# kyleliang919/distributed-lion-pytorch

Measured on AMD Instinct MI355X. Metric: tokens/sec + all-reduce bytes/step, GPT-2 CLM at 1/2/4/8 MI355X, higher is better.
Workload: dtype bf16; 1 GPU; model=gpt2 (124.4M params), trainable_params=124439808, base_weights=bf16, global_batch=160, task=clm, gradient_checkpointing=False, micro_batch=20, grad_accum=8, seq_len=1024, parallelism=dp1, optimizer=distributed Lion (majority vote), lr 0.0001, wd 0.1, exchange=a2a, impl=native

## Files before the change

### distributed_lion_pytorch_amd/csrc/bindings.cpp

```cpp
#include <ATen/ATen.h>
#include <c10/core/DeviceGuard.h>
#include <c10/hip/HIPStream.h>
#include <torch/library.h>

#include <hip/hip_runtime.h>

#include <cstdlib>
#include <string>
#include <tuple>
#include <vector>

#include "kernels.h"

namespace dlion {
enum class Layout : int { NT = 0, NN = 1, TN = 2, TT = 3 };
bool lt_gemm(const void* a, int64_t lda, const void* b, int64_t ldb, void* c, int64_t ldc, const void* bias,
             int64_t M, int64_t N, int64_t K, int epi, int device, hipStream_t s, Layout lay, bool accumulate);
}

namespace {

using at::Tensor;

void check_dev(const Tensor& t, const char* name) {
  TORCH_CHECK(t.is_cuda(), "dlion: ", name, " must be a GPU (HIP) tensor");
  TORCH_CHECK(t.is_contiguous(), "dlion: ", name, " must be contiguous");
}

void check_hip(hipError_t e, const char* what) {
  TORCH_CHECK(e == hipSuccess, "dlion: ", what, " failed: ", hipGetErrorString(e));
}

hipStream_t cur_stream() { return c10::hip::getCurrentHIPStream().stream(); }

const float* gscale_ptr(const std::optional<Tensor>& gscale) {
  if (!gscale.has_value()) return nullptr;
  check_dev(*gscale, "gscale");
  TORCH_CHECK(gscale->scalar_type() == at::kFloat && gscale->numel() >= 2, "dlion: gscale must be float32[2]");
  return gscale->data_ptr<float>();
}

void check_rounding(int64_t rounding, int64_t dtype, int64_t coord_base) {
  TORCH_CHECK(rounding == 0 || rounding == 1, "dlion: bad parameter rounding mode ", rounding);
  TORCH_CHECK(rounding == 0 || dtype != 2, "dlion: stochastic parameter rounding does not support fp16");
  TORCH_CHECK(coord_base >= 0 && coord_base % 8 == 0, "dlion: the coordinate base must be a multiple of 8");
}

void lion_local(const Tensor& meta, int64_t seg_off, int64_t chunk_off, int64_t n_chunks, int64_t dtype,
                double decay, double neg_lr, double b1, double omb1, double b2, double omb2,
                const std::optional<Tensor>& gscale, int64_t rounding, int64_t rkey, int64_t coord_base) {
  check_dev(meta, "meta");
  TORCH_CHECK(meta.scalar_type() == at::kLong, "dlion: meta must be int64");
  check_rounding(rounding, dtype, coord_base);
  const c10::DeviceGuard g(meta.device());
  const int64_t* base = meta.data_ptr<int64_t>();
  check_hip(dlion::launch_lion_local(static_cast<int>(dtype), base + seg_off, base + chunk_off, n_chunks,
                                     static_cast<float>(decay), static_cast<float>(neg_lr), static_cast<float>(b1),
                                     static_cast<float>(omb1), static_cast<float>(b2), static_cast<float>(omb2),
                                     gscale_ptr(gscale), cur_stream(), static_cast<int>(rounding),
                                     static_cast<uint32_t>(rkey), coord_base),
            "lion_local");
}

void lion_encode(const Tensor& meta, int64_t seg_off, int64_t chunk_off, int64_t n_chunks, int64_t dtype,
                 const Tensor& bits, double b1, double omb1, double b2, double omb2, bool update_m,
                 bool stochastic, double rr, int64_t seed, int64_t step, const std::optional<Tensor>& gscale,
                 int64_t cbase) {
  check_dev(meta, "meta");
  check_dev(bits, "bits");
  TORCH_CHECK(bits.scalar_type() == at::kByte, "dlion: bits must be uint8");
  TORCH_CHECK(cbase >= 0 && cbase % 8 == 0, "dlion: the coordinate base must be a multiple of 8");
  const c10::DeviceGuard g(meta.device());
  const int64_t* base = meta.data_ptr<int64_t>();
  check_hip(dlion::launch_lion_encode(static_cast<int>(dtype), base + seg_off, base + chunk_off, n_chunks,
                                      bits.data_ptr<uint8_t>(), static_cast<float>(b1), static_cast<float>(omb1),
                                      static_cast<float>(b2), static_cast<float>(omb2), update_m ? 1 : 0,
                                      stochastic ? 1 : 0, static_cast<float>(rr), static_cast<uint64_t>(seed),
                                      static_cast<uint32_t>(step), gscale_ptr(gscale), cur_stream(), cbase),
            "lion_encode");
}

void grad_sumsq(const Tensor& meta, int64_t seg_off, int64_t chunk_off, int64_t n_chunks, int64_t dtype,
                const Tensor& partial, int64_t part_off) {
  check_dev(meta, "meta");
  check_dev(partial, "partial");
  TORCH_CHECK(partial.scalar_type() == at::kFloat && part_off + n_chunks <= partial.numel(),
              "dlion: grad_sumsq partial buffer too small");
  const c10::DeviceGuard g(meta.device());
  const int64_t* base = meta.data_ptr<int64_t>();
  check_hip(dlion::launch_grad_sumsq(static_cast<int>(dtype), base + seg_off, base + chunk_off, n_chunks,
                                     partial.data_ptr<float>() + part_off, cur_stream()),
            "grad_sumsq");
}

void clip_coef(const Tensor& partial, int64_t n, double max_norm, const Tensor& out) {
  check_dev(partial, "partial");
  check_dev(out, "out");
  TORCH_CHECK(partial.scalar_type() == at::kFloat && out.scalar_type() == at::kFloat && out.numel() >= 2 &&
                  n <= partial.numel(),
              "dlion: clip_coef needs float32 partials and a float32[2] output");
  const c10::DeviceGuard g(partial.device());
  check_hip(dlion::launch_clip_coef(partial.data_ptr<float>(), n, static_cast<float>(max_norm), out.data_ptr<float>(),
                                    cur_stream()),
            "clip_coef");
}

void lion_vote_apply(const Tensor& meta, int64_t seg_off, int64_t chunk_off, int64_t n_chunks, int64_t dtype,
                     const Tensor& planes, int64_t plane_stride, const Tensor& alive, int64_t mode, int64_t tie,
                     const std::optional<Tensor>& neg, double decay, double neg_lr,
                     const std::optional<Tensor>& own, const std::optional<Tensor>& agree, int64_t rounding,
                     int64_t rkey, int64_t coord_base) {
  check_dev(meta, "meta");
  check_rounding(rounding, dtype, coord_base);
  check_dev(planes, "planes");
  check_dev(alive, "alive");
  TORCH_CHECK(planes.scalar_type() == at::kByte, "dlion: planes must be uint8");
  TORCH_CHECK(alive.scalar_type() == at::kByte, "dlion: alive must be uint8");
  TORCH_CHECK(mode >= 0 && mode <= 3, "dlion: bad vote mode ", mode);
  if (mode == 3) {
    const int64_t w = alive.numel();
    TORCH_CHECK(w >= 1 && w <= 15, "dlion: counted apply needs 1 <= W <= 15, got ", w);
    int64_t p = 0;
    while (w >> p) ++p;
    TORCH_CHECK(plane_stride > 0 && plane_stride % 256 == 0, "dlion: counted apply shard bytes must be a multiple of 256");
    TORCH_CHECK(planes.numel() >= w * p * plane_stride, "dlion: counted apply count planes too small");
  }
  const uint8_t* negp = nullptr;
  if (neg.has_value()) {
    check_dev(*neg, "neg");
    negp = neg->data_ptr<uint8_t>();
  }
  unsigned long long* agp = nullptr;
  const uint8_t* ownp = nullptr;
  if (agree.has_value()) {
    TORCH_CHECK(own.has_value(), "dlion: vote agreement needs this rank's own bits");
    check_dev(*own, "own");
    ownp = own->data_ptr<uint8_t>();
    check_dev(*agree, "agree");
    TORCH_CHECK(agree->scalar_type() == at::kLong && agree->numel() >= 2,
                "dlion: agree must be int64 [agreements, ties]");
    agp = reinterpret_cast<unsigned long long*>(agree->data_ptr<int64_t>());
  }
  const c10::DeviceGuard g(meta.device());
  const int64_t* base = meta.data_ptr<int64_t>();
  check_hip(dlion::launch_lion_vote_apply(static_cast<int>(dtype), base + seg_off, base + chunk_off, n_chunks,
                                          planes.data_ptr<uint8_t>(), plane_stride, alive.data_ptr<uint8_t>(),
                                          static_cast<int>(alive.numel()), static_cast<int>(mode),
                                          static_cast<int>(tie), negp, static_cast<float>(decay),
                                          static_cast<float>(neg_lr), ownp, agp, cur_stream(),
                                          static_cast<int>(rounding), static_cast<uint32_t>(rkey), coord_base),
            "lion_vote_apply");
}

void vote_reduce(const Tensor& recv, int64_t nbytes, const Tensor& alive, int64_t tie, const Tensor& out,
                 const std::optional<Tensor>& neg_out, const std::optional<Tensor>& ties) {
  check_dev(recv, "recv");
  check_dev(alive, "alive");
  check_dev(out, "out");
  TORCH_CHECK(nbytes % 4 == 0, "dlion: vote_reduce shard bytes must be a multiple of 4");
  TORCH_CHECK(out.numel() >= nbytes, "dlion: vote_reduce out too small");
  TORCH_CHECK(recv.numel() >= nbytes * alive.numel(), "dlion: vote_reduce recv too small");
  uint8_t* negp = nullptr;
  if (neg_out.has_value()) {
    check_dev(*neg_out, "neg_out");
    negp = neg_out->data_ptr<uint8_t>();
  }
  unsigned long long* tp = nullptr;
  if (ties.has_value()) {
    check_dev(*ties, "ties");
    TORCH_CHECK(ties->scalar_type() == at::kLong && ties->numel() >= 1, "dlion: ties must be int64");
    tp = reinterpret_cast<unsigned long long*>(ties->data_ptr<int64_t>());
  }
  const c10::DeviceGuard g(recv.device());
  check_hip(dlion::launch_vote_reduce(recv.data_ptr<uint8_t>(), nbytes, alive.data_ptr<uint8_t>(),
                                      static_cast<int>(alive.numel()), static_cast<int>(tie),
                                      out.data_ptr<uint8_t>(), negp, tp, cur_stream()),
            "vote_reduce");
}

void vote_count(const Tensor& recv, int64_t nbytes, const Tensor& alive, const Tensor& out,
                const std::optional<Tensor>& ties) {
  check_dev(recv, "recv");
  check_dev(alive, "alive");
  check_dev(out, "out");
  TORCH_CHECK(recv.scalar_type() == at::kByte && out.scalar_type() == at::kByte && alive.scalar_type() == at::kByte,
              "dlion: vote_count buffers must be uint8");
  const int64_t w = alive.numel();
  TORCH_CHECK(w >= 1 && w <= 15, "dlion: vote_count needs 1 <= W <= 15, got ", w);
  int64_t p = 0;
  while (w >> p) ++p;
  TORCH_CHECK(nbytes >= 0 && nbytes % 4 == 0, "dlion: vote_count shard bytes must be a multiple of 4");
  TORCH_CHECK(out.numel() >= p * nbytes, "dlion: vote_count out too small");
  TORCH_CHECK(recv.numel() >= nbytes * w, "dlion: vote_count recv too small");
  unsigned long long* tp = nullptr;
  if (ties.has_value()) {
    check_dev(*ties, "ties");
    TORCH_CHECK(ties->scalar_type() == at::kLong && ties->numel() >= 1, "dlion: ties must be int64");
    tp = reinterpret_cast<unsigned long long*>(ties->data_ptr<int64_t>());
  }
  const c10::DeviceGuard g(recv.device());
  check_hip(dlion::launch_vote_count(recv.data_ptr<uint8_t>(), nbytes, alive.data_ptr<uint8_t>(),
                                     static_cast<int>(w), out.data_ptr<uint8_t>(), tp, cur_stream()),
            "vote_count");
}

int dtype_code(at::ScalarType t) {
  switch (t) {
    case at::kFloat: return 0;
    case at::kBFloat16: return 1;
    case at::kHalf: return 2;
    default: TORCH_CHECK(false, "dlion: unsupported dtype ", t);
  }
  return -1;
}

Tensor softmax_xent_(const Tensor& logits, const Tensor& labels, int64_t v, int64_t variant) {
  check_dev(logits, "logits");
  check_dev(labels, "labels");
  TORCH_CHECK(logits.dim() == 2, "dlion: logits must be [N, Vpad]");
  TORCH_CHECK(labels.scalar_type() == at::kLong && labels.numel() == logits.size(0), "dlion: labels must be int64[N]");
  TORCH_CHECK(logits.size(1) % 8 == 0 && v <= logits.size(1), "dlion: padded vocab must be a multiple of 8");
  const c10::DeviceGuard g(logits.device());
  auto loss = at::empty({logits.size(0)}, logits.options().dtype(at::kFloat));
  check_hip(dlion::launch_softmax_xent(dtype_code(logits.scalar_type()), logits.data_ptr(), labels.data_ptr<int64_t>(),
                                       logits.size(0), logits.size(1), static_cast<int>(v), loss.data_ptr<float>(),
                                       static_cast<int>(variant), cur_stream()),
            "softmax_xent");
  return loss;
}

Tensor softmax_xent_opts_(const Tensor& logits, const Tensor& labels, int64_t v, double smoothing, double z_loss,
                          int64_t variant) {
  check_dev(logits, "logits");
  check_dev(labels, "labels");
  TORCH_CHECK(logits.dim() == 2 && logits.is_contiguous(), "dlion: logits must be a contiguous [N, Vpad]");
  TORCH_CHECK(labels.scalar_type() == at::kLong && labels.numel() == logits.size(0) && labels.is_contiguous(),
              "dlion: labels must be int64[N]");
  TORCH_CHECK(logits.size(1) % 8 == 0 && v > 0 && v <= logits.size(1), "dlion: padded vocab must be a multiple of 8");
  TORCH_CHECK(smoothing >= 0.0 && smoothing < 1.0 && z_loss >= 0.0, "dlion: need 0 <= smoothing < 1 and z_loss >= 0");
  const c10::DeviceGuard g(logits.device());
  auto loss = at::empty({logits.size(0)}, logits.options().dtype(at::kFloat));
  check_hip(dlion::launch_softmax_xent_opts(dtype_code(logits.scalar_type()), logits.data_ptr(),
                                            labels.data_ptr<int64_t>(), logits.size(0), logits.size(1),
                                            static_cast<int>(v), loss.data_ptr<float>(), static_cast<float>(smoothing),
                                            static_cast<float>(z_loss), static_cast<int>(variant), cur_stream()),
            "softmax_xent_opts");
  return loss;
}

std::tuple<Tensor, Tensor, Tensor, Tensor> lm_score(const Tensor& logits, const Tensor& labels, int64_t v,
                                                    double smoothing, double z_loss) {
  check_dev(logits, "logits");
  check_dev(labels, "labels");
  TORCH_CHECK(logits.dim() == 2 && logits.is_contiguous(), "dlion: logits must be a contiguous [N, Vpad]");
  TORCH_CHECK(labels.scalar_type() == at::kLong && labels.numel() == logits.size(0) && labels.is_contiguous(),
              "dlion: labels must be int64[N]");
  TORCH_CHECK(logits.size(1) % 8 == 0 && v > 0 && v <= logits.size(1), "dlion: padded vocab must be a multiple of 8");
  TORCH_CHECK(logits.size(1) <= (int64_t{1} << 30), "dlion: lm_score vocabulary too wide");
  TORCH_CHECK(smoothing >= 0.0 && smoothing < 1.0 && z_loss >= 0.0, "dlion: need 0 <= smoothing < 1 and z_loss >= 0");
  const c10::DeviceGuard g(logits.device());
  const int64_t n = logits.size(0);
  auto loss = at::empty({n}, logits.options().dtype(at::kFloat));
  auto lse = at::empty({n}, logits.options().dtype(at::kFloat));
  auto pred = at::empty({n}, logits.options().dtype(at::kInt));
  auto rank = at::empty({n}, logits.options().dtype(at::kInt));
  check_hip(dlion::launch_lm_score(dtype_code(logits.scalar_type()), logits.data_ptr(), labels.data_ptr<int64_t>(), n,
                                   logits.size(1), static_cast<int>(v), static_cast<float>(smoothing),
                                   static_cast<float>(z_loss), loss.data_ptr<float>(), lse.data_ptr<float>(),
                                   pred.data_ptr<int>(), rank.data_ptr<int>(), cur_stream()),
            "lm_score");
  return {loss, lse, pred, rank};
}

void check_bthd(const Tensor& t, const char* name) {
  TORCH_CHECK(t.is_cuda() && t.scalar_type() == at::kBFloat16, "dlion attn: ", name, " must be a bf16 GPU tensor");
  TORCH_CHECK(t.dim() == 4 && t.stride(3) == 1, "dlion attn: ", name, " must be [B,T,H,D] with contiguous D");
  TORCH_CHECK(reinterpret_cast<uintptr_t>(t.data_ptr()) % 16 == 0 && t.stride(1) % 8 == 0 && t.stride(2) % 8 == 0 &&
                  t.stride(0) % 8 == 0,
              "dlion attn: ", name, " must be 16-byte aligned");
}

dlion::AttnArgs attn_args(const Tensor& q, const Tensor& k, const Tensor& v, double p, int64_t seed) {
  check_bthd(q, "q");
  check_bthd(k, "k");
  check_bthd(v, "v");
  const int64_t B = q.size(0), T = q.size(1), H = q.size(2), D = q.size(3), Hkv = k.size(2);
  TORCH_CHECK(k.size(0) == B && k.size(1) == T && k.size(3) == D && v.sizes() == k.sizes(), "dlion attn: shape mismatch");
  TORCH_CHECK(H % Hkv == 0, "dlion attn: H must be a multiple of Hkv");
  TORCH_CHECK(T >= 1 && (D == 64 || D == 128), "dlion attn: need T >= 1 and D in {64, 128}");
  TORCH_CHECK(p >= 0.0 && p < 1.0, "dlion attn: dropout must be in [0, 1)");
  dlion::AttnArgs a{};
  a.q = static_cast<const __bf16*>(q.data_ptr());
  a.k = static_cast<const __bf16*>(k.data_ptr());
  a.v = static_cast<const __bf16*>(v.data_ptr());
  a.q_sb = q.stride(0); a.q_st = q.stride(1); a.q_sh = q.stride(2);
  a.k_sb = k.stride(0); a.k_st = k.stride(1); a.k_sh = k.stride(2);
  a.v_sb = v.stride(0); a.v_st = v.stride(1); a.v_sh = v.stride(2);
  a.B = static_cast<int>(B); a.T = static_cast<int>(T); a.H = static_cast<int>(H); a.Hkv = static_cast<int>(Hkv);
  a.scale = static_cast<float>(1.0 / std::sqrt(static_cast<double>(D)));
  a.scale_log2 = static_cast<float>(1.4426950408889634 / std::sqrt(static_cast<double>(D)));
  uint32_t th = static_cast<uint32_t>(std::llround(p * 65536.0));
  if (th > 65535u) th = 65535u;
  a.thresh16 = th;
  a.inv_keep = static_cast<float>(65536.0 / (65536.0 - th));
  a.seed = static_cast<uint32_t>(seed);
  return a;
}

void set_window(dlion::AttnArgs& a, int64_t window, int64_t D) {
  TORCH_CHECK(window >= 0, "dlion attn: window must be >= 0 (0 = plain causal)");
  a.window = window >= a.T ? 0 : static_cast<int>(window);
  TORCH_CHECK(a.window == 0 || D == 128, "dlion attn: a sliding window needs head_dim 128");
}

void set_bounds(dlion::AttnArgs& a, const std::optional<Tensor>& row_lo, const std::optional<Tensor>& key_hi,
                const Tensor& q) {
  a.row_lo = a.key_hi = nullptr;
  if (!row_lo.has_value() && !key_hi.has_value()) return;
  TORCH_CHECK(row_lo.has_value() && key_hi.has_value(), "dlion attn: row_lo and key_hi come as a pair");
  TORCH_CHECK(a.window == 0, "dlion attn: bounds replace the window (fold it into them)");
  TORCH_CHECK(q.size(3) == 128 && a.thresh16 == 0, "dlion attn: bounds need head_dim 128 and no dropout");
  for (const Tensor* t : {&*row_lo, &*key_hi}) {
    TORCH_CHECK(t->device() == q.device() && t->scalar_type() == at::kInt && t->is_contiguous() && t->dim() == 2 &&
                    t->size(0) == q.size(0) && t->size(1) == q.size(1),
                "dlion attn: row_lo / key_hi must be contiguous int32 [B, T] on the inputs' device");
  }
  a.row_lo = row_lo->data_ptr<int32_t>();
  a.key_hi = key_hi->data_ptr<int32_t>();
}

std::tuple<Tensor, Tensor> attn_fwd(const Tensor& q, const Tensor& k, const Tensor& v, double p, int64_t seed,
                                    int64_t window, const std::optional<Tensor>& row_lo,
                                    const std::optional<Tensor>& key_hi) {
  auto a = attn_args(q, k, v, p, seed);
  set_window(a, window, q.size(3));
  set_bounds(a, row_lo, key_hi, q);
  const c10::DeviceGuard g(q.device());
  auto out = at::empty({q.size(0), q.size(1), q.size(2), q.size(3)}, q.options());
  auto lse = at::empty({q.size(0), q.size(2), q.size(1)}, q.options().dtype(at::kFloat));
  a.out = static_cast<__bf16*>(out.data_ptr());
  a.o_sb = out.stride(0); a.o_st = out.stride(1); a.o_sh = out.stride(2);
  a.lse = lse.data_ptr<float>();
  check_hip(dlion::launch_attn_fwd(a, static_cast<int>(q.size(3)), a.thresh16 > 0, cur_stream()), "attn_fwd");
  return {out, lse};
}

void attn_bwd(const Tensor& q, const Tensor& k, const Tensor& v, const Tensor& out, const Tensor& dout,
              const Tensor& lse, double p, int64_t seed, const Tensor& dq, const Tensor& dk, const Tensor& dv,
              const std::optional<Tensor>& colsum, const std::optional<Tensor>& rope_cos,
              const std::optional<Tensor>& rope_sin, int64_t window, const std::optional<Tensor>& row_lo,
              const std::optional<Tensor>& key_hi) {
  auto a = attn_args(q, k, v, p, seed);
  set_window(a, window, q.size(3));
  set_bounds(a, row_lo, key_hi, q);
  TORCH_CHECK(a.row_lo == nullptr || !colsum.has_value(), "dlion attn: bounds do not go with bias-gradient partials");
  check_bthd(out, "out");
  check_bthd(dout, "dout");
  check_bthd(dq, "dq");
  check_bthd(dk, "dk");
  check_bthd(dv, "dv");
  TORCH_CHECK(out.strides() == dout.strides(), "dlion attn: out and dout must share strides");
  TORCH_CHECK(dk.strides() == dv.strides(), "dlion attn: dk and dv must share strides");
  TORCH_CHECK(lse.is_contiguous() && lse.scalar_type() == at::kFloat, "dlion attn: lse must be contiguous fp32");
  const c10::DeviceGuard g(q.device());
  auto delta = at::empty_like(lse);
  a.o = static_cast<const __bf16*>(out.data_ptr());
  a.dout = static_cast<const __bf16*>(dout.data_ptr());
  a.o_sb = out.stride(0); a.o_st = out.stride(1); a.o_sh = out.stride(2);
  a.lse = lse.data_ptr<float>();
  a.delta = delta.data_ptr<float>();
  a.dq = static_cast<__bf16*>(dq.data_ptr());
  a.dk = static_cast<__bf16*>(dk.data_ptr());
  a.dv = static_cast<__bf16*>(dv.data_ptr());
  a.dq_sb = dq.stride(0); a.dq_st = dq.stride(1); a.dq_sh = dq.stride(2);
  a.dk_sb = dk.stride(0); a.dk_st = dk.stride(1); a.dk_sh = dk.stride(2);
  a.colsum = nullptr;
  if (colsum.has_value()) {
    TORCH_CHECK(a.H == a.Hkv, "dlion attn: bias-gradient partials need H == Hkv");
    TORCH_CHECK(colsum->is_cuda() && colsum->scalar_type() == at::kFloat && colsum->is_contiguous() &&
                    colsum->dim() == 2 && colsum->size(0) == q.size(0) * ((q.size(1) + 31) / 32) &&
                    colsum->size(1) == 3 * q.size(2) * q.size(3),
                "dlion attn: colsum must be fp32 [B * ceil(T / 32), 3 * H * D]");
    a.colsum = colsum->data_ptr<float>();
  }
  a.rope_cos = a.rope_sin = nullptr;
  if (rope_cos.has_value() || rope_sin.has_value()) {
    TORCH_CHECK(rope_cos.has_value() && rope_sin.has_value() && !colsum.has_value(),
                "dlion attn: rope tables come as a pair, and not with bias-gradient partials");
    for (const Tensor* t : {&*rope_cos, &*rope_sin}) {
      TORCH_CHECK(t->is_cuda() && t->scalar_type() == at::kBFloat16 && t->is_contiguous() && t->dim() == 2 &&
                      t->size(0) >= q.size(1) && t->size(1) == q.size(3),
                  "dlion attn: rope tables must be contiguous bf16 [>= T, D]");
    }
    a.rope_cos = static_cast<const __bf16*>(rope_cos->data_ptr());
    a.rope_sin = static_cast<const __bf16*>(rope_sin->data_ptr());
  }
  check_hip(dlion::launch_attn_bwd(a, static_cast<int>(q.size(3)), a.thresh16 > 0, cur_stream()), "attn_bwd");
}

void check_rows(const Tensor& t, const char* name, int64_t C) {
  TORCH_CHECK(t.is_cuda() && t.scalar_type() == at::kBFloat16 && t.is_contiguous(), "dlion norm: ", name,
              " must be a contiguous bf16 GPU tensor");
  TORCH_CHECK(t.size(-1) == C, "dlion norm: ", name, " last dim mismatch");
}

void check_norm_width(int64_t C) {
  TORCH_CHECK(C >= 256 && C <= 8192 && C % 8 == 0,
              "dlion norm: hidden size must satisfy 256 <= C <= 8192 and C % 8 == 0, got ", C);
}

std::pair<uint32_t, float> drop_params(double p) {
  uint32_t th = static_cast<uint32_t>(std::llround(p * 65536.0));
  if (th > 65535u) th = 65535u;
  return {th, static_cast<float>(65536.0 / (65536.0 - th))};
}

std::tuple<Tensor, Tensor, Tensor, Tensor> add_norm_fwd(const Tensor& x, const std::optional<Tensor>& y,
                                                        const std::optional<Tensor>& bias, const Tensor& gamma,
                                                        const std::optional<Tensor>& beta, double eps, bool rms,
                                                        double p, int64_t seed) {
  const int64_t C = x.size(-1), rows = x.numel() / C;
  check_rows(x, "x", C);
  check_rows(gamma, "gamma", C);
  check_norm_width(C);
  TORCH_CHECK(rms || beta.has_value(), "dlion norm: LayerNorm needs beta");
  if (y.has_value()) check_rows(*y, "y", C);
  if (bias.has_value()) check_rows(*bias, "bias", C);
  const c10::DeviceGuard g(x.device());
  Tensor xo = y.has_value() ? at::empty_like(x) : x;
  Tensor h = at::empty_like(x);
  auto mean = at::empty({rows}, x.options().dtype(at::kFloat));
  auto rstd = at::empty({rows}, x.options().dtype(at::kFloat));
  const auto dp = drop_params(y.has_value() ? p : 0.0);
  check_hip(dlion::launch_add_norm_fwd(x.data_ptr(), y.has_value() ? y->data_ptr() : nullptr,
                                       bias.has_value() ? bias->data_ptr() : nullptr, gamma.data_ptr(),
                                       beta.has_value() ? beta->data_ptr() : nullptr, xo.data_ptr(), h.data_ptr(),
                                       mean.data_ptr<float>(), rstd.data_ptr<float>(), rows, static_cast<int>(C),
                                       static_cast<float>(eps), rms, static_cast<uint32_t>(seed), dp.first, dp.second,
                                       cur_stream()),
            "add_norm_fwd");
  return {xo, h, mean, rstd};
}

std::tuple<Tensor, Tensor, Tensor> add_norm_bwd(const Tensor& dh, const std::optional<Tensor>& dxo_in,
                                                const Tensor& xo, const Tensor& gamma, const Tensor& mean,
                                                const Tensor& rstd, bool rms, double p, int64_t seed, bool want_dy,
                                                int64_t parts) {
  const int64_t C = xo.size(-1), rows = xo.numel() / C;
  check_rows(dh, "dh", C);
  check_rows(xo, "xo", C);
  check_rows(gamma, "gamma", C);
  check_norm_width(C);
  if (dxo_in.has_value()) check_rows(*dxo_in, "dxo_in", C);
  const c10::DeviceGuard g(xo.device());
  auto dx = at::empty_like(xo);
  Tensor dy = want_dy ? at::empty_like(xo) : Tensor();
  TORCH_CHECK(parts >= 1 && parts <= 65535, "add_norm_bwd: parts out of range");
  auto part = at::empty({parts, 3, C}, xo.options().dtype(at::kFloat));
  const auto dp = drop_params(want_dy ? p : 0.0);
  check_hip(dlion::launch_add_norm_bwd(dh.data_ptr(), dxo_in.has_value() ? dxo_in->data_ptr() : nullptr, xo.data_ptr(),
                                       gamma.data_ptr(), mean.data_ptr<float>(), rstd.data_ptr<float>(), dx.data_ptr(),
                                       want_dy ? dy.data_ptr() : nullptr, part.data_ptr<float>(),
                                       static_cast<int>(parts), rows, static_cast<int>(C), rms,
                                       static_cast<uint32_t>(seed), dp.first, dp.second, cur_stream()),
            "add_norm_bwd");
  return {dx, dy, part};
}

Tensor bias_gelu_fwd(const Tensor& z, const Tensor& b, bool exact) {
  const int64_t N = z.size(-1), rows = z.numel() / N;
  check_rows(z, "z", N);
  check_rows(b, "b", N);
  TORCH_CHECK(N % 8 == 0 && N <= 16384, "dlion gelu: N must be a multiple of 8 and <= 16384");
  const c10::DeviceGuard g(z.device());
  auto h = at::empty_like(z);
  check_hip(dlion::launch_bias_gelu_fwd(z.data_ptr(), b.data_ptr(), h.data_ptr(), rows, static_cast<int>(N), exact,
                                        cur_stream()),
            "bias_gelu_fwd");
  return h;
}

std::tuple<Tensor, Tensor> bias_gelu_bwd(const Tensor& dh, const Tensor& z, const Tensor& b, bool exact,
                                         int64_t parts) {
  const int64_t N = z.size(-1), rows = z.numel() / N;
  check_rows(dh, "dh", N);
  check_rows(z, "z", N);
  check_rows(b, "b", N);
  const c10::DeviceGuard g(z.device());
  auto dz = at::empty_like(z);
  auto part = at::empty({parts, N}, z.options().dtype(at::kFloat));
  check_hip(dlion::launch_bias_gelu_bwd(dh.data_ptr(), z.data_ptr(), b.data_ptr(), dz.data_ptr(),
                                        part.data_ptr<float>(), static_cast<int>(parts), rows, static_cast<int>(N),
                                        exact, cur_stream()),
            "bias_gelu_bwd");
  return {dz, part};
}

struct Partials {
  const float* ptr;
  int64_t S, n, ld;
};
Partials partials(const Tensor& part) {
  TORCH_CHECK(part.is_cuda() && part.scalar_type() == at::kFloat, "dlion: partials must be fp32 on the GPU");
  TORCH_CHECK(reinterpret_cast<uintptr_t>(part.data_ptr()) % 16 == 0, "dlion: partials must be 16-byte aligned");
  if (part.is_contiguous()) return {part.data_ptr<float>(), part.size(0), part.numel() / part.size(0),
                                    part.numel() / part.size(0)};
  TORCH_CHECK(part.dim() == 2 && part.stride(1) == 1 && part.stride(0) % 4 == 0,
              "dlion: strided partials must be 2-D with unit column stride");
  return {part.data_ptr<float>(), part.size(0), part.size(1), part.stride(0)};
}

bool sum_partials_split(const std::vector<const float*>& ptrs, const std::vector<int64_t>& rows,
                        const std::vector<int64_t>& lds, int64_t n, void* out, bool accumulate, const float* scale,
                        const at::TensorOptions& opt) {
  int64_t total = 0;
  for (auto r : rows) total += r;
  const int Y = dlion::sum_partials_split_factor(n, total);
  if (Y <= 1) return false;
  auto scratch = at::empty({Y, n}, opt.dtype(at::kFloat));
  check_hip(dlion::launch_sum_partials_split(ptrs.data(), rows.data(), lds.data(), static_cast<int>(ptrs.size()), n, Y,
                                             scratch.data_ptr<float>(), out, accumulate, scale, cur_stream()),
            "sum_partials_split");
  return true;
}

bool sum_partials_split1(const Partials& P, void* out, bool accumulate, const float* scale,
                         const at::TensorOptions& opt) {
  return sum_partials_split({P.ptr}, {P.S}, {P.ld}, P.n, out, accumulate, scale, opt);
}

Tensor sum_partials(const Tensor& part) {
  const auto P = partials(part);
  TORCH_CHECK(P.n % 4 == 0, "dlion: partial row length must be a multiple of 4");
  const c10::DeviceGuard g(part.device());
  auto sizes = part.sizes().vec();
  sizes.erase(sizes.begin());
  auto out = at::empty(sizes, part.options().dtype(at::kBFloat16));
  if (sum_partials_split1(P, out.data_ptr(), false, nullptr, part.options())) return out;
  check_hip(dlion::launch_sum_partials(P.ptr, static_cast<int>(P.S), P.n, P.ld, out.data_ptr(), false, cur_stream()),
            "sum_partials");
  return out;
}

void sum_partials_acc_(const Tensor& part, const Tensor& out) {
  const auto P = partials(part);
  TORCH_CHECK(out.is_cuda() && out.scalar_type() == at::kBFloat16 && out.is_contiguous() && out.numel() == P.n,
              "dlion: accumulation target must be a contiguous bf16 tensor of the partial row size");
  TORCH_CHECK(P.n % 4 == 0, "dlion: partial row length must be a multiple of 4");
  const c10::DeviceGuard g(part.device());
  if (sum_partials_split1(P, out.data_ptr(), true, nullptr, part.options())) return;
  check_hip(dlion::launch_sum_partials(P.ptr, static_cast<int>(P.S), P.n, P.ld, out.data_ptr(), true, cur_stream()),
            "sum_partials_acc_");
}

void sum_partials_multi_(at::TensorList parts, const Tensor& out, bool accumulate) {
  TORCH_CHECK(!parts.empty() && parts.size() <= 16, "dlion: 1..16 partial stacks");
  std::vector<const float*> ptrs;
  std::vector<int64_t> rows, lds;
  int64_t n = -1;
  for (const auto& t : parts) {
    const auto P = partials(t);
    TORCH_CHECK(n < 0 || P.n == n, "dlion: partial stacks must have the same row length");
    n = P.n;
    ptrs.push_back(P.ptr);
    rows.push_back(P.S);
    lds.push_back(P.ld);
  }
  TORCH_CHECK(out.is_cuda() && out.scalar_type() == at::kBFloat16 && out.is_contiguous() && out.numel() == n,
              "dlion: target must be a contiguous bf16 tensor of the partial row size");
  TORCH_CHECK(n % 4 == 0, "dlion: partial row length must be a multiple of 4");
  const c10::DeviceGuard g(out.device());
  if (sum_partials_split(ptrs, rows, lds, n, out.data_ptr(), accumulate, nullptr, out.options())) return;
  check_hip(dlion::launch_sum_partials_multi(ptrs.data(), rows.data(), lds.data(), static_cast<int>(parts.size()), n,
                                             out.data_ptr(), accumulate, cur_stream()),
            "sum_partials_multi_");
}

void sum_partials_scaled_(const Tensor& part, const Tensor& s, const Tensor& out, bool accumulate) {
  const auto P = partials(part);
  check_dev(s, "s");
  TORCH_CHECK(s.scalar_type() == at::kFloat && s.numel() >= 1, "dlion: scale must be float32");
  TORCH_CHECK(out.is_cuda() && out.scalar_type() == at::kBFloat16 && out.is_contiguous() && out.numel() == P.n,
              "dlion: target must be a contiguous bf16 tensor of the partial row size");
  TORCH_CHECK(P.n % 4 == 0, "dlion: partial row length must be a multiple of 4");
  const c10::DeviceGuard g(part.device());
  if (sum_partials_split1(P, out.data_ptr(), accumulate, s.data_ptr<float>(), part.options())) return;
  check_hip(dlion::launch_sum_partials(P.ptr, static_cast<int>(P.S), P.n, P.ld, out.data_ptr(), accumulate, cur_stream(),
                                       s.data_ptr<float>()),
            "sum_partials_scaled_");
}

Tensor colsum_partials(const Tensor& x, int64_t parts) {
  TORCH_CHECK(x.is_cuda() && x.scalar_type() == at::kBFloat16 && x.is_contiguous(),
              "dlion colsum: x must be a contiguous bf16 GPU tensor");
  const int64_t N = x.size(-1), rows = x.numel() / N;
  TORCH_CHECK(N % 8 == 0 && N <= 16384 && parts >= 1 && parts <= 65535, "dlion colsum: bad shape");
  const c10::DeviceGuard g(x.device());
  auto part = at::empty({parts, N}, x.options().dtype(at::kFloat));
  check_hip(dlion::launch_colsum(x.data_ptr(), part.data_ptr<float>(), static_cast<int>(parts), rows,
                                 static_cast<int>(N), cur_stream()),
            "colsum");
  return part;
}

void rows_of(const Tensor& t, const char* what, int64_t& rows, int64_t& ld) {
  TORCH_CHECK(t.is_cuda() && t.scalar_type() == at::kBFloat16 && t.dim() >= 2 && t.stride(-1) == 1, "dlion ", what,
              ": operands must be bf16 GPU tensors [..., F] with unit column stride");
  ld = t.stride(-2);
  rows = 1;
  for (int64_t i = 0; i < t.dim() - 1; ++i) rows *= t.size(i);
  for (int64_t i = 0; i + 2 < t.dim(); ++i)
    TORCH_CHECK(t.size(i) == 1 || t.stride(i) == t.stride(i + 1) * t.size(i + 1), "dlion ", what,
                ": leading dims must collapse to rows of one stride");
  TORCH_CHECK(t.size(-1) % 8 == 0 && ld % 8 == 0 && reinterpret_cast<uintptr_t>(t.data_ptr()) % 16 == 0, "dlion ",
              what, ": F, the row stride and the base must be 16-byte aligned");
}

void check_pair(const Tensor& g, const Tensor& u, int64_t& rows, int64_t& ld) {
  rows_of(g, "swiglu", rows, ld);
  int64_t r2, ld2;
  rows_of(u, "swiglu", r2, ld2);
  TORCH_CHECK(g.sizes() == u.sizes() && ld == ld2, "dlion swiglu: gate / up shapes or strides differ");
}

Tensor swiglu_fwd(const Tensor& g, const Tensor& u) {
  int64_t rows, ld;
  check_pair(g, u, rows, ld);
  const c10::DeviceGuard dg(g.device());
  auto h = at::empty(g.sizes(), g.options());
  check_hip(dlion::launch_swiglu_fwd(g.data_ptr(), u.data_ptr(), h.data_ptr(), rows, g.size(-1), ld, cur_stream()),
            "swiglu_fwd");
  return h;
}

std::tuple<Tensor, Tensor> swiglu_bwd(const Tensor& dh, const Tensor& g, const Tensor& u) {
  int64_t rows, ld;
  check_pair(g, u, rows, ld);
  TORCH_CHECK(dh.is_contiguous() && dh.sizes() == g.sizes() && dh.scalar_type() == at::kBFloat16,
              "dlion swiglu: dh must be contiguous bf16 of the gate's shape");
  const c10::DeviceGuard dg(g.device());
  const int64_t F = g.size(-1);
  auto dgate = at::empty(g.sizes(), g.options()), dup = at::empty(g.sizes(), g.options());
  check_hip(dlion::launch_swiglu_bwd(dh.data_ptr(), g.data_ptr(), u.data_ptr(), dgate.data_ptr(), dup.data_ptr(),
                                     rows, F, ld, F, cur_stream()),
            "swiglu_bwd");
  return {dgate, dup};
}

Tensor swiglu_bwd_fused(const Tensor& dh, const Tensor& g, const Tensor& u) {
  int64_t rows, ld;
  check_pair(g, u, rows, ld);
  TORCH_CHECK(dh.is_contiguous() && dh.sizes() == g.sizes() && dh.scalar_type() == at::kBFloat16,
              "dlion swiglu: dh must be contiguous bf16 of the gate's shape");
  const c10::DeviceGuard dg(g.device());
  const int64_t F = g.size(-1);
  auto shape = g.sizes().vec();
  shape.back() = 2 * F;
  auto dgu = at::empty(shape, g.options());
  auto* base = static_cast<uint16_t*>(dgu.data_ptr());
  check_hip(dlion::launch_swiglu_bwd(dh.data_ptr(), g.data_ptr(), u.data_ptr(), base, base + F, rows, F, ld, 2 * F,
                                     cur_stream()),
            "swiglu_bwd_fused");
  return dgu;
}

std::tuple<Tensor, Tensor> swiglu_fwd_t(const Tensor& g, const Tensor& u) {
  int64_t rows, ld;
  check_pair(g, u, rows, ld);
  const int64_t F = g.size(-1);
  TORCH_CHECK(rows % 64 == 0 && F % 64 == 0, "dlion swiglu_fwd_t: rows and F must be multiples of 64");
  const c10::DeviceGuard dg(g.device());
  auto h = at::empty(g.sizes(), g.options());
  auto ht = at::empty({F, rows}, g.options());
  check_hip(dlion::launch_swiglu_fwd_t(g.data_ptr(), u.data_ptr(), h.data_ptr(), ht.data_ptr(), rows, F, ld,
                                       cur_stream()),
            "swiglu_fwd_t");
  return {h, ht};
}

std::tuple<Tensor, Tensor> swiglu_bwd_fused_t(const Tensor& dh, const Tensor& g, const Tensor& u) {
  int64_t rows, ld;
  check_pair(g, u, rows, ld);
  TORCH_CHECK(dh.is_contiguous() && dh.sizes() == g.sizes() && dh.scalar_type() == at::kBFloat16,
              "dlion swiglu: dh must be contiguous bf16 of the gate's shape");
  const int64_t F = g.size(-1);
  TORCH_CHECK(rows % 64 == 0 && F % 64 == 0, "dlion swiglu_bwd_fused_t: rows and F must be multiples of 64");
  const c10::DeviceGuard dg(g.device());
  auto shape = g.sizes().vec();
  shape.back() = 2 * F;
  auto dgu = at::empty(shape, g.options());
  auto dgut = at::empty({2 * F, rows}, g.options());
  check_hip(dlion::launch_swiglu_bwd_t(dh.data_ptr(), g.data_ptr(), u.data_ptr(), dgu.data_ptr(), dgut.data_ptr(),
                                       rows, F, ld, cur_stream()),
            "swiglu_bwd_fused_t");
  return {dgu, dgut};
}

Tensor rope(const Tensor& x, const Tensor& cos, const Tensor& sin, bool inverse) {
  TORCH_CHECK(x.dim() == 4 && x.is_cuda() && x.scalar_type() == at::kBFloat16, "dlion rope: x must be bf16 [B, T, H, D]");
  const int64_t B = x.size(0), T = x.size(1), H = x.size(2), D = x.size(3);
  TORCH_CHECK(x.stride(3) == 1 && x.stride(2) == D && (B == 1 || x.stride(0) == T * x.stride(1)) &&
                  x.stride(1) % 8 == 0 && reinterpret_cast<uintptr_t>(x.data_ptr()) % 16 == 0,
              "dlion rope: x must have contiguous heads and a uniform, 16-byte aligned token stride");
  TORCH_CHECK(D % 8 == 0, "dlion rope: head_dim must be a multiple of 8");
  for (const Tensor* t : {&cos, &sin})
    TORCH_CHECK(t->is_cuda() && t->scalar_type() == at::kBFloat16 && t->is_contiguous() && t->dim() == 2 &&
                    t->size(0) >= T && t->size(1) == D,
                "dlion rope: cos/sin must be contiguous bf16 [>=T, D]");
  const c10::DeviceGuard dg(x.device());
  auto y = at::empty(x.sizes(), x.options());
  check_hip(dlion::launch_rope(x.data_ptr(), cos.data_ptr(), sin.data_ptr(), y.data_ptr(), B * T,
                               static_cast<int>(T), static_cast<int>(H), static_cast<int>(D), inverse, x.stride(1),
                               H * D, cur_stream()),
            "rope");
  return y;
}

void rope_(const Tensor& x, const Tensor& cos, const Tensor& sin, bool inverse) {
  TORCH_CHECK(x.dim() == 4 && x.is_cuda() && x.scalar_type() == at::kBFloat16, "dlion rope_: x must be bf16 [B, T, H, D]");
  const int64_t B = x.size(0), T = x.size(1), H = x.size(2), D = x.size(3);
  TORCH_CHECK(x.stride(3) == 1 && x.stride(2) == D && (B == 1 || x.stride(0) == T * x.stride(1)) &&
                  x.stride(1) % 8 == 0 && reinterpret_cast<uintptr_t>(x.data_ptr()) % 16 == 0 && D % 8 == 0,
              "dlion rope_: x must have contiguous heads and a uniform, 16-byte aligned token stride");
  for (const Tensor* t : {&cos, &sin})
    TORCH_CHECK(t->is_cuda() && t->scalar_type() == at::kBFloat16 && t->is_contiguous() && t->dim() == 2 &&
                    t->size(0) >= T && t->size(1) == D,
                "dlion rope_: cos/sin must be contiguous bf16 [>=T, D]");
  const c10::DeviceGuard dg(x.device());
  check_hip(dlion::launch_rope(x.data_ptr(), cos.data_ptr(), sin.data_ptr(), x.data_ptr(), B * T,
                               static_cast<int>(T), static_cast<int>(H), static_cast<int>(D), inverse, x.stride(1),
                               x.stride(1), cur_stream()),
            "rope_");
}

int64_t qk_token_stride(const Tensor& x) { return x.size(1) == 1 && x.size(0) > 1 ? x.stride(0) : x.stride(1); }
bool qk_token_strided(const Tensor& x) {
  const int64_t B = x.size(0), T = x.size(1), D = x.size(3);
  return x.stride(3) == 1 && (x.size(2) == 1 || x.stride(2) == D) &&
         (B == 1 || T == 1 || x.stride(0) == T * x.stride(1)) && qk_token_stride(x) % 8 == 0 &&
         reinterpret_cast<uintptr_t>(x.data_ptr()) % 16 == 0;
}

void check_qk_norm(const char* what, const Tensor& x, const Tensor& gamma_a, const std::optional<Tensor>& gamma_b,
                   int64_t split, const Tensor* cos, const Tensor* sin) {
  TORCH_CHECK(x.dim() == 4 && x.is_cuda() && x.scalar_type() == at::kBFloat16, "dlion ", what,
              ": x must be bf16 [B, T, H, D]");
  const int64_t B = x.size(0), T = x.size(1), H = x.size(2), D = x.size(3);
  TORCH_CHECK(qk_token_strided(x), "dlion ", what,
              ": x must have contiguous heads and a uniform, 16-byte aligned token stride");
  TORCH_CHECK(D == 64 || D == 128, "dlion ", what, ": head_dim must be 64 or 128");
  TORCH_CHECK(split >= 0 && split <= H && (gamma_b.has_value() || split == H), "dlion ", what,
              ": split must lie in [0, H], and be H without gamma_b");
  for (const Tensor* g : {&gamma_a, gamma_b.has_value() ? &*gamma_b : &gamma_a})
    TORCH_CHECK(g->is_cuda() && g->scalar_type() == at::kBFloat16 && g->is_contiguous() && g->numel() == D &&
                    reinterpret_cast<uintptr_t>(g->data_ptr()) % 16 == 0,
                "dlion ", what, ": gains must be contiguous, 16-byte aligned bf16 [D]");
  TORCH_CHECK((cos == nullptr) == (sin == nullptr), "dlion ", what, ": cos/sin come as a pair");
  if (cos != nullptr)
    for (const Tensor* t : {cos, sin})
      TORCH_CHECK(t->is_cuda() && t->scalar_type() == at::kBFloat16 && t->is_contiguous() && t->dim() == 2 &&
                      t->size(0) >= T && t->size(1) == D,
                  "dlion ", what, ": cos/sin must be contiguous bf16 [>=T, D]");
}

std::tuple<Tensor, Tensor> qk_norm_rope_fwd(const Tensor& x, const Tensor& gamma_a,
                                            const std::optional<Tensor>& gamma_b, int64_t split, double eps,
                                            const Tensor& cos, const Tensor& sin) {
  check_qk_norm("qk_norm_rope_fwd", x, gamma_a, gamma_b, split, &cos, &sin);
  const int64_t B = x.size(0), T = x.size(1), H = x.size(2), D = x.size(3);
  const c10::DeviceGuard dg(x.device());
  auto y = at::empty(x.sizes(), x.options());
  auto rstd = at::empty({B, T, H}, x.options().dtype(at::kFloat));
  check_hip(dlion::launch_qk_norm_rope_fwd(x.data_ptr(), gamma_a.data_ptr(),
                                           (gamma_b.has_value() ? *gamma_b : gamma_a).data_ptr(), cos.data_ptr(),
                                           sin.data_ptr(), y.data_ptr(), rstd.data_ptr<float>(), B * T,
                                           static_cast<int>(T), static_cast<int>(H), static_cast<int>(D),
                                           static_cast<int>(split), static_cast<float>(eps), qk_token_stride(x), cur_stream()),
            "qk_norm_rope_fwd");
  return {y, rstd};
}

Tensor qk_norm_rope_bwd_(const Tensor& g, const Tensor& x, const Tensor& rstd, const Tensor& gamma_a,
                         const std::optional<Tensor>& gamma_b, int64_t split, const std::optional<Tensor>& cos,
                         const std::optional<Tensor>& sin, int64_t parts) {
  check_qk_norm("qk_norm_rope_bwd_", x, gamma_a, gamma_b, split, cos.has_value() ? &*cos : nullptr,
                sin.has_value() ? &*sin : nullptr);
  const int64_t B = x.size(0), T = x.size(1), H = x.size(2), D = x.size(3);
  TORCH_CHECK(g.dim() == 4 && g.is_cuda() && g.scalar_type() == at::kBFloat16 && g.sizes() == x.sizes() &&
                  qk_token_strided(g),
              "dlion qk_norm_rope_bwd_: g must be bf16 of x's shape with contiguous heads and a uniform, 16-byte "
              "aligned token stride");
  TORCH_CHECK(rstd.is_cuda() && rstd.scalar_type() == at::kFloat && rstd.is_contiguous() && rstd.numel() == B * T * H,
              "dlion qk_norm_rope_bwd_: rstd must be contiguous fp32 [B, T, H]");
  TORCH_CHECK(parts >= 1 && parts <= (1 << 20), "dlion qk_norm_rope_bwd_: parts out of range");
  const c10::DeviceGuard dg(x.device());
  auto part = at::empty({parts, 2, D}, x.options().dtype(at::kFloat));
  check_hip(dlion::launch_qk_norm_rope_bwd(g.data_ptr(), x.data_ptr(), rstd.data_ptr<float>(), gamma_a.data_ptr(),
                                           (gamma_b.has_value() ? *gamma_b : gamma_a).data_ptr(),
                                           cos.has_value() ? cos->data_ptr() : nullptr,
                                           sin.has_value() ? sin->data_ptr() : nullptr, part.data_ptr<float>(),
                                           static_cast<int>(parts), B * T, static_cast<int>(T), static_cast<int>(H),
                                           static_cast<int>(D), static_cast<int>(split), qk_token_stride(g), qk_token_stride(x),
                                           cur_stream()),
            "qk_norm_rope_bwd_");
  return part;
}

void check_gemm_operand(const Tensor& t, const char* name) {
  TORCH_CHECK(t.is_cuda() && t.scalar_type() == at::kBFloat16 && t.dim() == 2 && t.stride(1) == 1,
              "dlion gemm: ", name, " must be a 2-D bf16 GPU tensor with unit column stride");
  TORCH_CHECK(t.stride(0) % 8 == 0 && reinterpret_cast<uintptr_t>(t.data_ptr()) % 16 == 0,
              "dlion gemm: ", name, " rows must be 16-byte aligned");
}

bool gemm_nt_supported(const Tensor& a, const Tensor& b) {
  return a.dim() == 2 && b.dim() == 2 && a.size(1) == b.size(1) && a.size(1) % 128 == 0 && b.size(0) % 8 == 0 &&
         a.size(0) * a.stride(0) < (1ll << 31) && b.size(0) * b.stride(0) < (1ll << 31);
}

void gemm_nt_launch(const Tensor& a, const Tensor& b, const Tensor& c, const Tensor* bias, const Tensor* aux,
                    int64_t epi, const Tensor* part = nullptr) {
  check_gemm_operand(a, "a");
  check_gemm_operand(b, "b");
  check_gemm_operand(c, "out");
  TORCH_CHECK(gemm_nt_supported(a, b), "dlion gemm: unsupported shape a=", a.sizes(), " b=", b.sizes(),
              " (needs K % 128 == 0, N % 8 == 0)");
  TORCH_CHECK(c.size(0) == a.size(0) && c.size(1) == b.size(0), "dlion gemm: output shape mismatch");
  if (bias) {
    TORCH_CHECK(bias->is_cuda() && bias->scalar_type() == at::kBFloat16 && bias->is_contiguous() &&
                    bias->numel() == b.size(0),
                "dlion gemm: bias must be a contiguous bf16 [N] tensor");
  }
  if (aux) {
    check_gemm_operand(*aux, "aux");
    TORCH_CHECK(aux->size(0) == c.size(0) && aux->size(1) == c.size(1), "dlion gemm: aux must match the output shape");
  }
  if (part) {
    TORCH_CHECK(part->is_cuda() && part->scalar_type() == at::kFloat && part->is_contiguous() &&
                    part->size(0) == 2 * ((a.size(0) + 255) / 256) && part->size(1) == b.size(0),
                "dlion gemm: part must be fp32 [2 * ceil(M / 256), N]");
  }
  const c10::DeviceGuard g(a.device());
  check_hip(dlion::launch_gemm_nt(a.data_ptr(), static_cast<int>(a.stride(0)), b.data_ptr(),
                                  static_cast<int>(b.stride(0)), c.data_ptr(), static_cast<int>(c.stride(0)),
                                  bias ? bias->data_ptr() : nullptr, aux ? aux->data_ptr() : nullptr,
                                  aux ? static_cast<int>(aux->stride(0)) : 0, static_cast<int>(a.size(0)),
                                  static_cast<int>(b.size(0)), static_cast<int>(a.size(1)), static_cast<int>(epi),
                                  part ? part->data_ptr<float>() : nullptr, cur_stream()),
            "gemm_nt");
}

Tensor gemm_nt(const Tensor& a, const Tensor& b, const std::optional<Tensor>& bias) {
  auto c = at::empty({a.size(0), b.size(0)}, a.options());
  gemm_nt_launch(a, b, c, bias.has_value() ? &*bias : nullptr, nullptr, bias.has_value() ? 1 : 0);
  return c;
}

void gemm_nt_out(const Tensor& a, const Tensor& b, const std::optional<Tensor>& bias, const Tensor& out) {
  gemm_nt_launch(a, b, out, bias.has_value() ? &*bias : nullptr, nullptr, bias.has_value() ? 1 : 0);
}

std::tuple<Tensor, Tensor> gemm_nt_gelu(const Tensor& a, const Tensor& b, const Tensor& bias, bool exact) {
  auto h = at::empty({a.size(0), b.size(0)}, a.options());
  auto z = at::empty_like(h);
  gemm_nt_launch(a, b, h, &bias, &z, exact ? 3 : 2);
  return {h, z};
}

bool lt_gemm_nt(const Tensor& a, const Tensor& b, const std::optional<Tensor>& bias, int64_t epi, const Tensor& out) {
  check_gemm_operand(a, "a");
  check_gemm_operand(b, "b");
  check_gemm_operand(out, "out");
  TORCH_CHECK(epi >= 0 && epi <= 2, "dlion lt_gemm: bad epilogue ", epi);
  TORCH_CHECK(a.size(1) == b.size(1) && out.size(0) == a.size(0) && out.size(1) == b.size(0),
              "dlion lt_gemm: shape mismatch a=", a.sizes(), " b=", b.sizes(), " out=", out.sizes());
  TORCH_CHECK(bias.has_value() == (epi != 0), "dlion lt_gemm: epilogue ", epi, epi ? " needs" : " takes no", " bias");
  if (bias.has_value()) {
    TORCH_CHECK(bias->is_cuda() && bias->scalar_type() == at::kBFloat16 && bias->is_contiguous() &&
                    bias->numel() == b.size(0),
                "dlion lt_gemm: bias must be a contiguous bf16 [N] tensor");
  }
  const c10::DeviceGuard g(a.device());
  return dlion::lt_gemm(a.data_ptr(), a.stride(0), b.data_ptr(), b.stride(0), out.data_ptr(), out.stride(0),
                        bias.has_value() ? bias->data_ptr() : nullptr, a.size(0), b.size(0), a.size(1),
                        static_cast<int>(epi), a.device().index(), cur_stream(), dlion::Layout::NT, false);
}

bool lt_gemm_nn(const Tensor& a, const Tensor& b, const Tensor& out) {
  check_gemm_operand(a, "a");
  check_gemm_operand(b, "b");
  check_gemm_operand(out, "out");
  TORCH_CHECK(a.size(1) == b.size(0) && out.size(0) == a.size(0) && out.size(1) == b.size(1),
              "dlion lt_gemm_nn: shape mismatch a=", a.sizes(), " b=", b.sizes(), " out=", out.sizes());
  const c10::DeviceGuard g(a.device());
  return dlion::lt_gemm(a.data_ptr(), a.stride(0), b.data_ptr(), b.stride(0), out.data_ptr(), out.stride(0), nullptr,
                        a.size(0), b.size(1), a.size(1), 0, a.device().index(), cur_stream(), dlion::Layout::NN, false);
}

bool lt_gemm_nt_acc(const Tensor& a, const Tensor& b, const Tensor& out, bool accumulate) {
  check_gemm_operand(a, "a");
  check_gemm_operand(b, "b");
  check_gemm_operand(out, "out");
  TORCH_CHECK(a.size(1) == b.size(1) && out.size(0) == a.size(0) && out.size(1) == b.size(0),
              "dlion lt_gemm_nt_acc: shape mismatch a=", a.sizes(), " b=", b.sizes(), " out=", out.sizes());
  const c10::DeviceGuard g(a.device());
  return dlion::lt_gemm(a.data_ptr(), a.stride(0), b.data_ptr(), b.stride(0), out.data_ptr(), out.stride(0), nullptr,
                        a.size(0), b.size(0), a.size(1), 0, a.device().index(), cur_stream(), dlion::Layout::NT,
                        accumulate);
}

bool lt_gemm_layout(const Tensor& a, const Tensor& b, const Tensor& out, int64_t layout, bool accumulate) {
  check_gemm_operand(a, "a");
  check_gemm_operand(b, "b");
  check_gemm_operand(out, "out");
  TORCH_CHECK(layout >= 0 && layout <= 3, "dlion lt_gemm_layout: layout must be 0..3");
  const bool at = layout >= 2, bt = layout == 0 || layout == 3;
  const int64_t M = at ? a.size(1) : a.size(0), K = at ? a.size(0) : a.size(1), N = bt ? b.size(0) : b.size(1);
  TORCH_CHECK((bt ? b.size(1) : b.size(0)) == K && out.size(0) == M && out.size(1) == N,
              "dlion lt_gemm_layout: shape mismatch a=", a.sizes(), " b=", b.sizes(), " out=", out.sizes(),
              " layout ", layout);
  const c10::DeviceGuard g(a.device());
  return dlion::lt_gemm(a.data_ptr(), a.stride(0), b.data_ptr(), b.stride(0), out.data_ptr(), out.stride(0), nullptr,
                        M, N, K, 0, a.device().index(), cur_stream(), static_cast<dlion::Layout>(layout), accumulate);
}

bool lt_gemm_tn(const Tensor& a, const Tensor& b, const Tensor& out, bool accumulate) {
  check_gemm_operand(a, "a");
  check_gemm_operand(b, "b");
  check_gemm_operand(out, "out");
  TORCH_CHECK(a.size(0) == b.size(0) && out.size(0) == a.size(1) && out.size(1) == b.size(1),
              "dlion lt_gemm_tn: shape mismatch a=", a.sizes(), " b=", b.sizes(), " out=", out.sizes());
  const c10::DeviceGuard g(a.device());
  return dlion::lt_gemm(a.data_ptr(), a.stride(0), b.data_ptr(), b.stride(0), out.data_ptr(), out.stride(0), nullptr,
                        a.size(1), b.size(1), a.size(0), 0, a.device().index(), cur_stream(), dlion::Layout::TN,
                        accumulate);
}

void check_bf16_contig(const Tensor& t, const char* name) {
  TORCH_CHECK(t.is_cuda() && t.scalar_type() == at::kBFloat16 && t.is_contiguous() &&
                  reinterpret_cast<uintptr_t>(t.data_ptr()) % 16 == 0,
              "dlion embed: ", name, " must be a contiguous, 16-byte aligned bf16 GPU tensor");
}

int32_t* err_ptr(const std::optional<Tensor>& err, const Tensor& like) {
  if (!err.has_value()) return nullptr;
  TORCH_CHECK(err->scalar_type() == at::kInt && err->numel() >= 1 && err->device() == like.device(),
              "dlion: the index-error flag must be an int32 tensor on the ids' device");
  return err->data_ptr<int32_t>();
}

void index_check_(const Tensor& ids, int64_t hi, int64_t ignore, const Tensor& err, int64_t code) {
  check_dev(ids, "ids");
  TORCH_CHECK(ids.scalar_type() == at::kLong && ids.is_contiguous(), "dlion index_check: ids must be contiguous int64");
  const c10::DeviceGuard g(ids.device());
  check_hip(dlion::launch_index_check(ids.data_ptr<int64_t>(), ids.numel(), hi, ignore, err_ptr(err, ids),
                                      static_cast<int>(code), cur_stream()),
            "index_check");
}

Tensor embed_fwd(const Tensor& ids, const Tensor& wte, const Tensor& wpe, double p, int64_t seed,
                 const std::optional<Tensor>& err) {
  check_dev(ids, "ids");
  TORCH_CHECK(ids.scalar_type() == at::kLong && ids.dim() == 2, "dlion embed: ids must be int64 [B, T]");
  check_bf16_contig(wte, "wte");
  check_bf16_contig(wpe, "wpe");
  const int64_t C = wte.size(1), T = ids.size(1);
  TORCH_CHECK(wpe.size(1) == C && T <= wpe.size(0) && C % 8 == 0, "dlion embed: shape mismatch / C % 8 != 0");
  TORCH_CHECK(p >= 0.0 && p < 1.0, "dlion embed: dropout must be in [0, 1)");
  const c10::DeviceGuard g(ids.device());
  auto out = at::empty({ids.size(0), T, C}, wte.options());
  const auto dp = drop_params(p);
  check_hip(dlion::launch_embed_fwd(ids.data_ptr<int64_t>(), wte.data_ptr(), wpe.data_ptr(), out.data_ptr(), ids.numel(),
                                    static_cast<int>(C), static_cast<int>(T), wte.size(0), static_cast<uint32_t>(seed),
                                    dp.first, dp.second, err_ptr(err, ids), cur_stream()),
            "embed_fwd");
  return out;
}

void embed_bwd_(const Tensor& dx, const std::optional<Tensor>& sid, const std::optional<Tensor>& perm,
                const std::optional<Tensor>& dwte, const std::optional<Tensor>& dwpe, int64_t T, bool pos_accumulate,
                double p, int64_t seed) {
  check_bf16_contig(dx, "dx");
  const int64_t C = dx.size(-1), n = dx.numel() / C;
  TORCH_CHECK(T > 0 && n % T == 0 && C % 8 == 0, "dlion embed: dx must be [B*T, C] with C % 8 == 0");
  int64_t V = 0;
  if (dwte.has_value()) {
    check_bf16_contig(*dwte, "dwte");
    TORCH_CHECK(dwte->dim() == 2 && dwte->size(1) == C, "dlion embed: dwte must be [V, C]");
    TORCH_CHECK(sid.has_value() && perm.has_value() && sid->numel() == n && perm->numel() == n &&
                    sid->scalar_type() == at::kLong && perm->scalar_type() == at::kLong && sid->is_contiguous() &&
                    perm->is_contiguous(),
                "dlion embed: the token gradient needs sorted ids and their permutation (int64 [n])");
    V = dwte->size(0);
  }
  if (dwpe.has_value()) {
    check_bf16_contig(*dwpe, "dwpe");
    TORCH_CHECK(dwpe->size(-1) == C && dwpe->size(0) >= T, "dlion embed: dwpe must be [>= T, C]");
  }
  const c10::DeviceGuard g(dx.device());
  const auto dp = drop_params(p);
  check_hip(dlion::launch_embed_bwd(dx.data_ptr(), dwte.has_value() ? sid->data_ptr<int64_t>() : nullptr,
                                    dwte.has_value() ? perm->data_ptr<int64_t>() : nullptr,
                                    dwte.has_value() ? dwte->data_ptr() : nullptr,
                                    dwpe.has_value() ? dwpe->data_ptr() : nullptr, n, static_cast<int>(C),
                                    static_cast<int>(T), V, pos_accumulate ? 1 : 0, static_cast<uint32_t>(seed),
                                    dp.first, dp.second, cur_stream()),
            "embed_bwd");
}

void scale_acc_(const Tensor& x, const Tensor& s, const Tensor& y, bool accumulate) {
  check_bf16_contig(x, "x");
  check_bf16_contig(y, "y");
  check_dev(s, "s");
  TORCH_CHECK(s.scalar_type() == at::kFloat && s.numel() >= 1, "dlion scale_acc: s must be float32");
  TORCH_CHECK(x.numel() == y.numel() && x.numel() % 8 == 0, "dlion scale_acc: size mismatch / numel % 8 != 0");
  const c10::DeviceGuard g(x.device());
  check_hip(dlion::launch_scale_acc(x.data_ptr(), s.data_ptr<float>(), y.data_ptr(), x.numel(), accumulate ? 1 : 0,
                                    cur_stream()),
            "scale_acc");
}

Tensor gemm_nt_stamped(const Tensor& a, const Tensor& b, const Tensor& stamps) {
  check_gemm_operand(a, "a");
  check_gemm_operand(b, "b");
  TORCH_CHECK(gemm_nt_supported(a, b), "dlion gemm: unsupported shape");
  const int64_t blocks = ((a.size(0) + 255) / 256) * ((b.size(0) + 255) / 256);
  TORCH_CHECK(stamps.is_cuda() && stamps.scalar_type() == at::kLong && stamps.is_contiguous() &&
                  stamps.numel() >= blocks * 8,
              "dlion gemm: stamps must be int64 [blocks, 8]");
  auto c = at::empty({a.size(0), b.size(0)}, a.options());
  const c10::DeviceGuard g(a.device());
  check_hip(dlion::launch_gemm_nt_stamped(a.data_ptr(), static_cast<int>(a.stride(0)), b.data_ptr(),
                                          static_cast<int>(b.stride(0)), c.data_ptr(), static_cast<int>(c.stride(0)),
                                          static_cast<int>(a.size(0)), static_cast<int>(b.size(0)),
                                          static_cast<int>(a.size(1)),
                                          reinterpret_cast<unsigned long long*>(stamps.data_ptr<int64_t>()),
                                          cur_stream()),
            "gemm_nt_stamped");
  return c;
}

std::tuple<Tensor, Tensor> gemm_nt_gelu_d(const Tensor& a, const Tensor& b, const Tensor& bias, bool exact) {
  auto h = at::empty({a.size(0), b.size(0)}, a.options());
  auto d = at::empty({a.size(0), b.size(0)}, a.options());
  gemm_nt_launch(a, b, h, &bias, &d, exact ? 7 : 6);
  return {h, d};
}

std::tuple<Tensor, Tensor> gemm_nt_dmul(const Tensor& a, const Tensor& b, const Tensor& d) {
  auto dz = at::empty({a.size(0), b.size(0)}, a.options());
  auto part = at::empty({2 * ((a.size(0) + 255) / 256), b.size(0)}, a.options().dtype(at::kFloat));
  gemm_nt_launch(a, b, dz, nullptr, &d, 8, &part);
  return {dz, part};
}

std::tuple<Tensor, Tensor> gemm_nt_dgelu(const Tensor& a, const Tensor& b, const Tensor& bias, const Tensor& z,
                                         bool exact) {
  auto dz = at::empty({a.size(0), b.size(0)}, a.options());
  auto part = at::empty({2 * ((a.size(0) + 255) / 256), b.size(0)}, a.options().dtype(at::kFloat));
  gemm_nt_launch(a, b, dz, &bias, &z, exact ? 5 : 4, &part);
  return {dz, part};
}

void gemm_tn_check_launch(at::TensorList P, at::TensorList Q, int64_t splits, const Tensor& out, bool accumulate) {
  TORCH_CHECK(!P.empty() && P.size() == Q.size() && P.size() <= 16, "dlion gemm_tn: 1..16 segment pairs");
  const int64_t rows = P[0].size(0), M = P[0].size(1), N = Q[0].size(1);
  const int64_t ldp = P[0].stride(0), ldq = Q[0].stride(0);
  std::vector<const void*> pp, qq;
  for (size_t i = 0; i < P.size(); ++i) {
    for (const Tensor* t : {&P[i], &Q[i]}) {
      TORCH_CHECK(t->is_cuda() && t->scalar_type() == at::kBFloat16 && t->dim() == 2 && t->stride(1) == 1 &&
                      reinterpret_cast<uintptr_t>(t->data_ptr()) % 16 == 0,
                  "dlion gemm_tn: operands must be 2-D bf16 GPU tensors with unit column stride, 16-byte aligned");
    }
    TORCH_CHECK(P[i].size(0) == rows && Q[i].size(0) == rows && P[i].size(1) == M && Q[i].size(1) == N &&
                    P[i].stride(0) == ldp && Q[i].stride(0) == ldq,
                "dlion gemm_tn: every segment must have the same shape and row stride");
    pp.push_back(P[i].data_ptr());
    qq.push_back(Q[i].data_ptr());
  }
  TORCH_CHECK(rows % 128 == 0 && M % 8 == 0 && N % 8 == 0 && ldp % 8 == 0 && ldq % 8 == 0,
              "dlion gemm_tn: rows % 128, M % 8, N % 8 and row strides % 8 must be 0");
  TORCH_CHECK(splits >= 1 && splits <= static_cast<int64_t>(P.size()) * rows / 128, "dlion gemm_tn: bad split count");
  const bool bf16_out = out.scalar_type() == at::kBFloat16;
  if (bf16_out) {
    TORCH_CHECK(splits == 1 && out.is_cuda() && out.is_contiguous() && out.numel() == M * N &&
                    reinterpret_cast<uintptr_t>(out.data_ptr()) % 8 == 0,
                "dlion gemm_tn: a bf16 out must be one contiguous [M, N] (unsplit) tensor");
  } else {
    TORCH_CHECK(out.is_cuda() && out.scalar_type() == at::kFloat && out.is_contiguous() && out.dim() == 3 &&
                    out.size(0) == splits && out.size(1) == M && out.size(2) == N,
                "dlion gemm_tn: out must be a contiguous fp32 [splits, M, N] tensor");
  }
  const c10::DeviceGuard g(P[0].device());
  check_hip(dlion::launch_gemm_tn(pp.data(), qq.data(), static_cast<int>(P.size()), rows, static_cast<int>(ldp),
                                  static_cast<int>(ldq), bf16_out ? nullptr : out.data_ptr<float>(),
                                  static_cast<int>(M), static_cast<int>(N), static_cast<int>(splits), accumulate,
                                  cur_stream(), bf16_out ? out.data_ptr() : nullptr),
            "gemm_tn");
}

Tensor gemm_tn(at::TensorList P, at::TensorList Q, int64_t splits) {
  TORCH_CHECK(!P.empty() && !Q.empty(), "dlion gemm_tn: no operands");
  auto out = at::empty({splits, P[0].size(1), Q[0].size(1)}, P[0].options().dtype(at::kFloat));
  gemm_tn_check_launch(P, Q, splits, out, false);
  return out;
}

void gemm_tn_(at::TensorList P, at::TensorList Q, const Tensor& out, bool accumulate) {
  if (out.scalar_type() == at::kBFloat16) {
    gemm_tn_check_launch(P, Q, 1, out, accumulate);
    return;
  }
  TORCH_CHECK(out.dim() == 3, "dlion gemm_tn_: out must be [splits, M, N]");
  gemm_tn_check_launch(P, Q, out.size(0), out, accumulate);
}

bool lora_rank_ok(int64_t r) { return r == 8 || r == 16 || dlion::lora_wide_rank(static_cast<int>(r)); }

void check_lora_rows(const Tensor& t, const char* name) {
  TORCH_CHECK(t.is_cuda() && t.scalar_type() == at::kBFloat16 && t.dim() == 2 && t.stride(1) == 1 &&
                  t.stride(0) % 8 == 0 && t.size(1) % 8 == 0 && reinterpret_cast<uintptr_t>(t.data_ptr()) % 16 == 0,
              "dlion lora: ", name, " must be a 2-D bf16 GPU tensor, unit column stride, row stride and width % 8 == 0");
}

Tensor lora_rows(const Tensor& x, const Tensor& w, double scale, double p, int64_t seed) {
  check_lora_rows(x, "x");
  check_bf16_contig(w, "w");
  const int64_t r = w.size(0);
  TORCH_CHECK(w.dim() == 2 && w.size(1) == x.size(1) && lora_rank_ok(r) && x.size(1) % 32 == 0,
              "dlion lora: w must be [8|16|32|64|128, K] with K % 32 == 0");
  const c10::DeviceGuard g(x.device());
  auto u = at::empty({x.size(0), r}, x.options());
  const auto dp = drop_params(p);
  const auto launch = dlion::lora_wide_rank(static_cast<int>(r)) ? dlion::launch_lora_rows_wide : dlion::launch_lora_rows;
  check_hip(launch(x.data_ptr(), x.stride(0), w.data_ptr(), u.data_ptr(), x.size(0), static_cast<int>(x.size(1)),
                   static_cast<int>(r), static_cast<float>(scale), static_cast<uint32_t>(seed), dp.first, dp.second,
                   cur_stream()),
            "lora_rows");
  return u;
}

Tensor lora_up(const Tensor& o, const Tensor& u, const Tensor& b, double s) {
  check_lora_rows(o, "o");
  check_bf16_contig(u, "u");
  check_bf16_contig(b, "b");
  const int64_t r = u.size(1);
  TORCH_CHECK(u.dim() == 2 && u.size(0) == o.size(0) && b.dim() == 2 && b.size(0) == o.size(1) && b.size(1) == r &&
                  lora_rank_ok(r),
              "dlion lora: shape mismatch (u [M, r], b [N, r], r in {8, 16, 32, 64, 128})");
  const c10::DeviceGuard g(o.device());
  auto out = at::empty({o.size(0), o.size(1)}, o.options());
  const auto launch = dlion::lora_wide_rank(static_cast<int>(r)) ? dlion::launch_lora_up_wide : dlion::launch_lora_up;
  check_hip(launch(o.data_ptr(), o.stride(0), u.data_ptr(), b.data_ptr(), out.data_ptr(), o.size(0),
                   static_cast<int>(o.size(1)), static_cast<int>(r), static_cast<float>(s), cur_stream()),
            "lora_up");
  return out;
}

std::tuple<Tensor, Tensor> lora_cols(const Tensor& g, const Tensor& y, const std::optional<Tensor>& a, double yscale,
                                     double p, int64_t seed) {
  check_lora_rows(g, "g");
  check_bf16_contig(y, "y");
  const int64_t r = y.size(1), M = g.size(0), N = g.size(1);
  TORCH_CHECK(y.dim() == 2 && y.size(0) == M && lora_rank_ok(r), "dlion lora: y must be [M, 8|16|32|64|128]");
  const bool mode1 = a.has_value();
  if (mode1) {
    check_bf16_contig(*a, "a");
    TORCH_CHECK(a->dim() == 2 && a->size(0) == r && a->size(1) == N, "dlion lora: a must be [r, N]");
  }
  const c10::DeviceGuard dg(g.device());
  const bool wide = dlion::lora_wide_rank(static_cast<int>(r));
  const int parts = wide ? dlion::lora_cols_parts_wide(M, static_cast<int>(N), static_cast<int>(r))
                         : dlion::lora_cols_parts(M, static_cast<int>(N));
  const auto launch = wide ? dlion::launch_lora_cols_wide : dlion::launch_lora_cols;
  auto part = mode1 ? at::empty({parts, r, N}, g.options().dtype(at::kFloat))
                    : at::empty({parts, N, r}, g.options().dtype(at::kFloat));
  Tensor dx = mode1 ? at::empty({M, N}, g.options()) : Tensor();
  const auto dp = drop_params(mode1 ? p : 0.0);
  check_hip(launch(g.data_ptr(), g.stride(0), y.data_ptr(), mode1 ? a->data_ptr() : nullptr,
                   mode1 ? dx.data_ptr() : nullptr, part.data_ptr<float>(), M, static_cast<int>(N), static_cast<int>(r),
                   parts, mode1 ? 1 : 0, static_cast<float>(yscale), static_cast<uint32_t>(seed), dp.first, dp.second,
                   cur_stream()),
            "lora_cols");
  return {part, dx};
}


std::tuple<Tensor, Tensor> quant4(const Tensor& w, const Tensor& code) {
  check_dev(w, "w");
  check_dev(code, "code");
  TORCH_CHECK(code.scalar_type() == at::kFloat && code.numel() == 16, "dlion quant4: code must be float32[16]");
  const int64_t n = w.numel();
  TORCH_CHECK(n % 64 == 0, "dlion quant4: numel must be a multiple of 64, got ", n);
  TORCH_CHECK(w.is_contiguous() && reinterpret_cast<uintptr_t>(w.data_ptr()) % 16 == 0,
              "dlion quant4: w must be contiguous and 16-byte aligned (the kernel reads it as flat vectors)");
  const c10::DeviceGuard g(w.device());
  auto q = at::empty({n / 2}, w.options().dtype(at::kByte));
  auto absmax = at::empty({n / 64}, w.options().dtype(at::kFloat));
  check_hip(dlion::launch_quant4(dtype_code(w.scalar_type()), w.data_ptr(), code.data_ptr<float>(),
                                 q.data_ptr<uint8_t>(), absmax.data_ptr<float>(), n, cur_stream()),
            "quant4");
  return {q, absmax};
}

void dequant4_(const Tensor& q, const Tensor& absmax, const Tensor& code, const Tensor& out) {
  check_dev(q, "q");
  check_dev(absmax, "absmax");
  check_dev(code, "code");
  check_dev(out, "out");
  TORCH_CHECK(q.scalar_type() == at::kByte && absmax.scalar_type() == at::kFloat && code.scalar_type() == at::kFloat &&
                  code.numel() == 16,
              "dlion dequant4: q uint8, absmax / code float32");
  const int64_t n = out.numel();
  TORCH_CHECK(n % 64 == 0 && q.numel() == n / 2 && absmax.numel() == n / 64,
              "dlion dequant4: out numel ", n, " does not match q ", q.numel(), " / absmax ", absmax.numel());
  TORCH_CHECK(reinterpret_cast<uintptr_t>(q.data_ptr()) % 16 == 0 && reinterpret_cast<uintptr_t>(out.data_ptr()) % 16 == 0,
              "dlion dequant4: q and out must be 16-byte aligned");
  TORCH_CHECK(out.is_contiguous() && q.is_contiguous() && absmax.is_contiguous(),
              "dlion dequant4: q, absmax and out must be contiguous (out is written linearly)");
  const c10::DeviceGuard g(out.device());
  check_hip(dlion::launch_dequant4(dtype_code(out.scalar_type()), q.data_ptr<uint8_t>(), absmax.data_ptr<float>(),
                                   code.data_ptr<float>(), out.data_ptr(), n, cur_stream()),
            "dequant4");
}

Tensor transpose_pad(const Tensor& x, int64_t rows_out) {
  TORCH_CHECK(x.is_cuda() && x.dim() == 2 && x.stride(1) == 1 && x.element_size() == 2,
              "dlion transpose_pad: x must be a 2-D 16-bit GPU tensor with unit column stride");
  const int64_t R = x.size(0), C = x.size(1);
  const int64_t Rp = rows_out < 0 ? R : rows_out;
  TORCH_CHECK(Rp >= R && Rp % 8 == 0 && x.stride(0) % 8 == 0 && reinterpret_cast<uintptr_t>(x.data_ptr()) % 16 == 0,
              "dlion transpose_pad: needs rows_out >= rows, rows_out % 8 == 0, row stride % 8 == 0, 16-byte alignment");
  const c10::DeviceGuard g(x.device());
  auto out = at::empty({C, Rp}, x.options());
  check_hip(dlion::launch_transpose_pad(x.data_ptr(), R, C, x.stride(0), out.data_ptr(), Rp, cur_stream()),
            "transpose_pad");
  return out;
}

void dequant4_t_(const Tensor& q, const Tensor& absmax, const Tensor& code, const Tensor& out) {
  check_dev(q, "q");
  check_dev(absmax, "absmax");
  check_dev(code, "code");
  TORCH_CHECK(out.is_cuda() && out.dim() == 2 && out.stride(1) == 1 && out.element_size() == 2,
              "dlion dequant4_t: out must be a 2-D 16-bit GPU view with unit column stride");
  const int64_t K = out.size(0), N = out.size(1);
  TORCH_CHECK(q.scalar_type() == at::kByte && q.numel() * 2 == N * K && absmax.numel() * 64 == N * K &&
                  code.numel() == 16 && code.scalar_type() == at::kFloat,
              "dlion dequant4_t: q / absmax do not match out");
  const c10::DeviceGuard g(out.device());
  check_hip(dlion::launch_dequant4_t(dtype_code(out.scalar_type()), q.data_ptr<uint8_t>(), absmax.data_ptr<float>(),
                                     code.data_ptr<float>(), out.data_ptr(), static_cast<int>(N), static_cast<int>(K),
                                     out.stride(0), cur_stream()),
            "dequant4_t");
}
}

TORCH_LIBRARY(dlion, m) {
  m.def("dequant4_t_(Tensor q, Tensor absmax, Tensor code, Tensor(a!) out) -> ()");
  m.def("transpose_pad(Tensor x, int rows_out=-1) -> Tensor");
  m.def("quant4(Tensor w, Tensor code) -> (Tensor, Tensor)");
  m.def("dequant4_(Tensor q, Tensor absmax, Tensor code, Tensor(a!) out) -> ()");
  m.def("gemm_tn(Tensor[] P, Tensor[] Q, int splits) -> Tensor");
  m.def("gemm_tn_(Tensor[] P, Tensor[] Q, Tensor(a!) out, bool accumulate) -> ()");
  m.def("lora_rows(Tensor x, Tensor w, float scale, float p, int seed) -> Tensor");
  m.def("lora_up(Tensor o, Tensor u, Tensor b, float s) -> Tensor");
  m.def("lora_cols(Tensor g, Tensor y, Tensor? a, float yscale, float p, int seed) -> (Tensor, Tensor)");
  m.def("gemm_nt_dgelu(Tensor a, Tensor b, Tensor bias, Tensor z, bool exact) -> (Tensor, Tensor)");
  m.def("gemm_nt_gelu_d(Tensor a, Tensor b, Tensor bias, bool exact) -> (Tensor, Tensor)");
  m.def("gemm_nt_dmul(Tensor a, Tensor b, Tensor d) -> (Tensor, Tensor)");
  m.def("gemm_nt_stamped(Tensor a, Tensor b, Tensor(a!) stamps) -> Tensor");
  m.def("embed_fwd(Tensor ids, Tensor wte, Tensor wpe, float p, int seed, Tensor(a!)? err=None) -> Tensor");
  m.def("index_check_(Tensor ids, int hi, int ignore, Tensor(a!) err, int code) -> ()");
  m.def(
      "embed_bwd_(Tensor dx, Tensor? sid, Tensor? perm, Tensor(a!)? dwte, Tensor(b!)? dwpe, int T, bool pos_accumulate,"
      " float p, int seed) -> ()");
  m.def("scale_acc_(Tensor x, Tensor s, Tensor(a!) y, bool accumulate) -> ()");
  m.def("lt_gemm_nt(Tensor a, Tensor b, Tensor? bias, int epi, Tensor(a!) out) -> bool");
  m.def("lt_gemm_nn(Tensor a, Tensor b, Tensor(a!) out) -> bool");
  m.def("lt_gemm_tn(Tensor a, Tensor b, Tensor(a!) out, bool accumulate) -> bool");
  m.def("lt_gemm_nt_acc(Tensor a, Tensor b, Tensor(a!) out, bool accumulate) -> bool");
  m.def("lt_gemm_layout(Tensor a, Tensor b, Tensor(a!) out, int layout, bool accumulate) -> bool");
  m.def("gemm_nt(Tensor a, Tensor b, Tensor? bias) -> Tensor");
  m.def("gemm_nt_out(Tensor a, Tensor b, Tensor? bias, Tensor(a!) out) -> ()");
  m.def("gemm_nt_gelu(Tensor a, Tensor b, Tensor bias, bool exact) -> (Tensor, Tensor)");
  m.def("swiglu_fwd(Tensor g, Tensor u) -> Tensor");
  m.def("swiglu_bwd(Tensor dh, Tensor g, Tensor u) -> (Tensor, Tensor)");
  m.def("swiglu_bwd_fused(Tensor dh, Tensor g, Tensor u) -> Tensor");
  m.def("swiglu_bwd_fused_t(Tensor dh, Tensor g, Tensor u) -> (Tensor, Tensor)");
  m.def("swiglu_fwd_t(Tensor g, Tensor u) -> (Tensor, Tensor)");
  m.def("rope(Tensor x, Tensor cos, Tensor sin, bool inverse) -> Tensor");
  m.def("rope_(Tensor(a!) x, Tensor cos, Tensor sin, bool inverse) -> ()");
  m.def("qk_norm_rope_fwd(Tensor x, Tensor gamma_a, Tensor? gamma_b, int split, float eps, Tensor cos, Tensor sin)"
        " -> (Tensor, Tensor)");
  m.def("qk_norm_rope_bwd_(Tensor(a!) g, Tensor x, Tensor rstd, Tensor gamma_a, Tensor? gamma_b, int split,"
        " Tensor? cos, Tensor? sin, int parts) -> Tensor");
  m.def(
      "add_norm_fwd(Tensor x, Tensor? y, Tensor? bias, Tensor gamma, Tensor? beta, float eps, bool rms, float p,"
      " int seed) -> (Tensor, Tensor, Tensor, Tensor)");
  m.def(
      "add_norm_bwd(Tensor dh, Tensor? dxo_in, Tensor xo, Tensor gamma, Tensor mean, Tensor rstd, bool rms,"
      " float p, int seed, bool want_dy, int parts) -> (Tensor, Tensor, Tensor)");
  m.def("bias_gelu_fwd(Tensor z, Tensor b, bool exact) -> Tensor");
  m.def("bias_gelu_bwd(Tensor dh, Tensor z, Tensor b, bool exact, int parts) -> (Tensor, Tensor)");
  m.def("sum_partials(Tensor part) -> Tensor");
  m.def("sum_partials_acc_(Tensor part, Tensor(a!) out) -> ()");
  m.def("sum_partials_scaled_(Tensor part, Tensor s, Tensor(a!) out, bool accumulate) -> ()");
  m.def("sum_partials_multi_(Tensor[] parts, Tensor(a!) out, bool accumulate) -> ()");
  m.def("colsum_partials(Tensor x, int parts) -> Tensor");
  m.def("attn_fwd(Tensor q, Tensor k, Tensor v, float p, int seed, int window=0, Tensor? row_lo=None,"
        " Tensor? key_hi=None) -> (Tensor, Tensor)");
  m.def(
      "attn_bwd(Tensor q, Tensor k, Tensor v, Tensor out, Tensor dout, Tensor lse, float p, int seed,"
      " Tensor(a!) dq, Tensor(b!) dk, Tensor(c!) dv, Tensor(d!)? colsum=None, Tensor? rope_cos=None,"
      " Tensor? rope_sin=None, int window=0, Tensor? row_lo=None, Tensor? key_hi=None) -> ()");
  m.def("softmax_xent_(Tensor(a!) logits, Tensor labels, int v, int variant=0) -> Tensor");
  m.def("softmax_xent_opts_(Tensor(a!) logits, Tensor labels, int v, float smoothing, float z_loss, int variant=0) -> Tensor");
  m.def("lm_score(Tensor logits, Tensor labels, int v, float smoothing, float z_loss) -> (Tensor, Tensor, Tensor, Tensor)");
  m.def(
      "lion_local(Tensor meta, int seg_off, int chunk_off, int n_chunks, int dtype, float decay, float neg_lr,"
      " float b1, float omb1, float b2, float omb2, Tensor? gscale=None, int rounding=0, int rkey=0,"
      " int coord_base=0) -> ()");
  m.def(
      "lion_encode(Tensor meta, int seg_off, int chunk_off, int n_chunks, int dtype, Tensor(a!) bits, float b1,"
      " float omb1, float b2, float omb2, bool update_m, bool stochastic, float rr, int seed, int step,"
      " Tensor? gscale=None, int cbase=0) -> ()");
  m.def("grad_sumsq(Tensor meta, int seg_off, int chunk_off, int n_chunks, int dtype, Tensor(a!) partial,"
        " int part_off) -> ()");
  m.def("clip_coef(Tensor partial, int n, float max_norm, Tensor(a!) out) -> ()");
  m.def(
      "lion_vote_apply(Tensor meta, int seg_off, int chunk_off, int n_chunks, int dtype, Tensor planes,"
      " int plane_stride, Tensor alive, int mode, int tie, Tensor? neg, float decay, float neg_lr,"
      " Tensor? own, Tensor(b!)? agree, int rounding=0, int rkey=0, int coord_base=0) -> ()");
  m.def("vote_reduce(Tensor recv, int nbytes, Tensor alive, int tie, Tensor(a!) out, Tensor(b!)? neg_out,"
        " Tensor(c!)? ties=None) -> ()");
  m.def("vote_count(Tensor recv, int nbytes, Tensor alive, Tensor(a!) out, Tensor(b!)? ties) -> ()");
}

TORCH_LIBRARY_IMPL(dlion, CUDA, m) {
  m.impl("lion_local", &lion_local);
  m.impl("lion_encode", &lion_encode);
  m.impl("lion_vote_apply", &lion_vote_apply);
  m.impl("vote_reduce", &vote_reduce);
  m.impl("vote_count", &vote_count);
  m.impl("grad_sumsq", &grad_sumsq);
  m.impl("clip_coef", &clip_coef);
  m.impl("softmax_xent_", &softmax_xent_);
  m.impl("softmax_xent_opts_", &softmax_xent_opts_);
  m.impl("lm_score", &lm_score);
  m.impl("attn_fwd", &attn_fwd);
  m.impl("attn_bwd", &attn_bwd);
  m.impl("add_norm_fwd", &add_norm_fwd);
  m.impl("add_norm_bwd", &add_norm_bwd);
  m.impl("bias_gelu_fwd", &bias_gelu_fwd);
  m.impl("bias_gelu_bwd", &bias_gelu_bwd);
  m.impl("sum_partials", &sum_partials);
  m.impl("sum_partials_acc_", &sum_partials_acc_);
  m.impl("sum_partials_scaled_", &sum_partials_scaled_);
  m.impl("sum_partials_multi_", &sum_partials_multi_);
  m.impl("colsum_partials", &colsum_partials);
  m.impl("swiglu_fwd", &swiglu_fwd);
  m.impl("swiglu_bwd", &swiglu_bwd);
  m.impl("swiglu_bwd_fused", &swiglu_bwd_fused);
  m.impl("swiglu_bwd_fused_t", &swiglu_bwd_fused_t);
  m.impl("swiglu_fwd_t", &swiglu_fwd_t);
  m.impl("rope", &rope);
  m.impl("rope_", &rope_);
  m.impl("qk_norm_rope_fwd", &qk_norm_rope_fwd);
  m.impl("qk_norm_rope_bwd_", &qk_norm_rope_bwd_);
  m.impl("gemm_nt", &gemm_nt);
  m.impl("gemm_nt_out", &gemm_nt_out);
  m.impl("gemm_nt_gelu", &gemm_nt_gelu);
  m.impl("gemm_nt_dgelu", &gemm_nt_dgelu);
  m.impl("gemm_nt_gelu_d", &gemm_nt_gelu_d);
  m.impl("gemm_nt_dmul", &gemm_nt_dmul);
  m.impl("gemm_nt_stamped", &gemm_nt_stamped);
  m.impl("embed_fwd", &embed_fwd);
  m.impl("index_check_", &index_check_);
  m.impl("embed_bwd_", &embed_bwd_);
  m.impl("scale_acc_", &scale_acc_);
  m.impl("lt_gemm_nt", &lt_gemm_nt);
  m.impl("lt_gemm_nn", &lt_gemm_nn);
  m.impl("lt_gemm_tn", &lt_gemm_tn);
  m.impl("lt_gemm_nt_acc", &lt_gemm_nt_acc);
  m.impl("lt_gemm_layout", &lt_gemm_layout);
  m.impl("gemm_tn", &gemm_tn);
  m.impl("gemm_tn_", &gemm_tn_);
  m.impl("lora_rows", &lora_rows);
  m.impl("lora_up", &lora_up);
  m.impl("lora_cols", &lora_cols);
  m.impl("quant4", &quant4);
  m.impl("dequant4_", &dequant4_);
  m.impl("dequant4_t_", &dequant4_t_);
  m.impl("transpose_pad", &transpose_pad);
}
```

### distributed_lion_pytorch_amd/csrc/gemm.hip

```cpp
#include "common.h"

#include <algorithm>

namespace dlion {

namespace {

typedef __bf16 bf16x8 __attribute__((ext_vector_type(8)));
typedef float f32x4 __attribute__((ext_vector_type(4)));

constexpr int kBM = 256, kBN = 256, kBK = 64;
constexpr int kHalf = 128 * kBK * 2;
constexpr int kLds = 8 * kHalf;

struct GemmArgs {
  const uint16_t* A;
  const uint16_t* B;
  uint16_t* C;
  const uint16_t* bias;
  uint16_t* aux;
  float* part;
  unsigned long long* stamps;
  int lda, ldb, ldc, ldaux;
  int M, N, K;
  int tiles_m, tiles_n;
};

__device__ __forceinline__ constexpr int slot(int dbuf, int ab, int half) { return ((dbuf * 2 + ab) * 2 + half) * kHalf; }

__device__ __forceinline__ void vm_wait6() { asm volatile("s_waitcnt vmcnt(6)" ::: "memory"); }
__device__ __forceinline__ void vm_wait8() { asm volatile("s_waitcnt vmcnt(8)" ::: "memory"); }
__device__ __forceinline__ void vm_wait2() { asm volatile("s_waitcnt vmcnt(2)" ::: "memory"); }
__device__ __forceinline__ void vm_wait0() { asm volatile("s_waitcnt vmcnt(0)" ::: "memory"); }

__device__ __forceinline__ void glds16(const uint16_t* base, uint32_t boff, uint8_t* dst) {
  const uint8_t* src = reinterpret_cast<const uint8_t*>(base) + boff;
  __builtin_amdgcn_global_load_lds((const __attribute__((address_space(1))) void*)src,
                                   (__attribute__((address_space(3))) void*)dst, 16, 0, 0);
}

typedef unsigned int u32x4 __attribute__((ext_vector_type(4)));
template <bool NT, typename V>
__device__ __forceinline__ void st16(uint16_t* p, const V& v) {
  const u32x4 x = __builtin_bit_cast(u32x4, v);
  if constexpr (NT) __builtin_nontemporal_store(x, reinterpret_cast<u32x4*>(p));
  else *reinterpret_cast<u32x4*>(p) = x;
}
template <bool NT>
__device__ __forceinline__ uint4 ld16(const uint16_t* p) {
  u32x4 x;
  if constexpr (NT) x = __builtin_nontemporal_load(reinterpret_cast<const u32x4*>(p));
  else x = *reinterpret_cast<const u32x4*>(p);
  return make_uint4(x[0], x[1], x[2], x[3]);
}
constexpr bool kNtAux = true, kNtC = true;

__device__ __forceinline__ f32x4 mfma16(const bf16x8& a, const bf16x8& b, const f32x4& c) {
  return __builtin_amdgcn_mfma_f32_16x16x32_bf16(a, b, c, 0, 0, 0);
}

struct Stage {
  uint32_t off[2][2][2];
};

#define DLION_STAMP(dst)                                                            \
  if constexpr (STAMP) {                                                            \
    __builtin_amdgcn_sched_barrier(0);                                              \
    asm volatile("s_memtime %0\n\ts_waitcnt lgkmcnt(0)" : "=s"(dst) :: "memory");    \
    __builtin_amdgcn_sched_barrier(0);                                              \
  }
#define DLION_RSTAMP(dst)                                                           \
  if constexpr (STAMP) {                                                            \
    __builtin_amdgcn_sched_barrier(0);                                              \
    asm volatile("s_memrealtime %0\n\ts_waitcnt lgkmcnt(0)" : "=s"(dst) :: "memory"); \
    __builtin_amdgcn_sched_barrier(0);                                              \
  }

template <int EPI, bool STAMP = false>
__global__ void __launch_bounds__(512, 1) gemm_nt_kernel(const GemmArgs g) {
  unsigned long long st_[7] = {0, 0, 0, 0, 0, 0, 0};
  DLION_RSTAMP(st_[5])
  DLION_STAMP(st_[0])
  __shared__ __attribute__((aligned(16))) uint8_t lds[kLds];

  const int tid = threadIdx.x;
  const int w = __builtin_amdgcn_readfirstlane(tid >> 6), lane = tid & 63;
  const int wr = w >> 2, wc = w & 3;

  const int nwg = g.tiles_m * g.tiles_n;
  const int bid = blockIdx.x;
  const int xcd = bid & 7, q8 = nwg >> 3, r8 = nwg & 7;
  const int wg = (xcd < r8 ? xcd * (q8 + 1) : r8 * (q8 + 1) + (xcd - r8) * q8) + (bid >> 3);
  constexpr int GM = 8;
  const int per_group = GM * g.tiles_n;
  const int grp = wg / per_group;
  const int first_m = grp * GM;
  const int gsz = min(g.tiles_m - first_m, GM);
  const int in_g = wg - grp * per_group;
  const int tm = first_m + in_g % gsz;
  const int tn = in_g / gsz;
  const int m0 = tm * kBM, n0 = tn * kBN;

  Stage st;
  {
    const int pc = lane & 7;
#pragma unroll
    for (int pi = 0; pi < 2; ++pi) {
      const int q = 2 * w + pi;
      const int lr = 8 * q + (lane >> 3);
      const int c = pc ^ ((lr >> 1) & 7);
#pragma unroll
      for (int h = 0; h < 2; ++h) {
        const int ra = min(m0 + (lr >> 6) * 128 + 64 * h + (lr & 63), g.M - 1);
        st.off[0][h][pi] = static_cast<uint32_t>(ra * g.lda + c * 8) * 2u;
        const int rb = min(n0 + 128 * h + lr, g.N - 1);
        st.off[1][h][pi] = static_cast<uint32_t>(rb * g.ldb + c * 8) * 2u;
      }
    }
  }
  const uint16_t* __restrict__ Ag = g.A;
  const uint16_t* __restrict__ Bg = g.B;

  auto stage = [&](int ab, int half, int dbuf, int kt) {
    const uint16_t* base = (ab == 0 ? Ag : Bg) + kt * kBK;
    asm volatile("" : "+s"(base));
    uint8_t* dst = lds + slot(dbuf, ab, half) + (2 * w) * 1024;
    asm volatile("" : "+v"(st.off[ab][half][0]), "+v"(st.off[ab][half][1]));
    glds16(base, st.off[ab][half][0], dst);
    glds16(base, st.off[ab][half][1], dst + 1024);
  };

  const int lr16 = lane & 15;
  const int swz = (lr16 >> 1) & 7;
  const int foff0 = lr16 * 128 + (((lane >> 4) ^ swz) << 4);
  const int foff1 = lr16 * 128 + (((4 + (lane >> 4)) ^ swz) << 4);
  const int a_row_base = wr * 64 * 128;
  const int b_base_off = ((wc >> 1) * kHalf) + (wc & 1) * 64 * 128;

  f32x4 acc[8][4];
#pragma unroll
  for (int i = 0; i < 8; ++i)
#pragma unroll
    for (int j = 0; j < 4; ++j) acc[i][j] = f32x4{0.f, 0.f, 0.f, 0.f};

  bf16x8 bfr[4][2];
  bf16x8 afr[2][2];

  auto read_b = [&](int dbuf) {
    const uint8_t* base = lds + slot(dbuf, 1, 0) + b_base_off;
#pragma unroll
    for (int nt = 0; nt < 4; ++nt) {
      bfr[nt][0] = *reinterpret_cast<const bf16x8*>(base + nt * 16 * 128 + foff0);
      bfr[nt][1] = *reinterpret_cast<const bf16x8*>(base + nt * 16 * 128 + foff1);
    }
  };
  auto read_a = [&](int dbuf, int p) {
    const uint8_t* base = lds + slot(dbuf, 0, p >> 1) + a_row_base + (2 * (p & 1)) * 16 * 128;
#pragma unroll
    for (int mt = 0; mt < 2; ++mt) {
      afr[mt][0] = *reinterpret_cast<const bf16x8*>(base + mt * 16 * 128 + foff0);
      afr[mt][1] = *reinterpret_cast<const bf16x8*>(base + mt * 16 * 128 + foff1);
    }
  };

#define DLION_GEMM_MFMA(P)                                                       \
  do {                                                                           \
    __builtin_amdgcn_s_setprio(1);                                               \
    _Pragma("unroll") for (int mt = 0; mt < 2; ++mt)                             \
    _Pragma("unroll") for (int nt = 0; nt < 4; ++nt)                             \
    _Pragma("unroll") for (int s = 0; s < 2; ++s)                                \
      acc[2 * (P) + mt][nt] = mfma16(bfr[nt][s], afr[mt][s], acc[2 * (P) + mt][nt]); \
    __builtin_amdgcn_s_setprio(0);                                               \
  } while (0)

#define DLION_GEMM_PHASE_MATH(P)                     \
  __builtin_amdgcn_s_barrier();                      \
  asm volatile("s_waitcnt lgkmcnt(0)" ::: "memory"); \
  __builtin_amdgcn_sched_barrier(0);                 \
  DLION_GEMM_MFMA(P);                                \
  __builtin_amdgcn_sched_barrier(0);                 \
  __builtin_amdgcn_s_barrier();

  const int nk = g.K / kBK;
  const int nit = nk / 2;

  stage(1, 0, 0, 0);
  stage(1, 1, 0, 0);
  stage(0, 0, 0, 0);
  stage(0, 1, 0, 0);
  stage(1, 0, 1, 1);
  stage(1, 1, 1, 1);
  vm_wait6();
  __builtin_amdgcn_s_barrier();
  if (wr == 1) __builtin_amdgcn_s_barrier();
  DLION_STAMP(st_[1])

  for (int it = 0; it < nit; ++it) {
    const int kt = 2 * it;
    const bool more = it + 1 < nit;
    read_b(0);
    read_a(0, 0);
    stage(0, 0, 1, kt + 1);
    DLION_GEMM_PHASE_MATH(0)
    read_a(0, 1);
    stage(0, 1, 1, kt + 1);
    vm_wait8();
    DLION_GEMM_PHASE_MATH(1)
    read_a(0, 2);
    if (more) stage(1, 0, 0, kt + 2);
    DLION_GEMM_PHASE_MATH(2)
    read_a(0, 3);
    if (more) {
      stage(1, 1, 0, kt + 2);
      vm_wait6();
    } else {
      vm_wait2();
    }
    DLION_GEMM_PHASE_MATH(3)
    read_b(1);
    read_a(1, 0);
    if (more) stage(0, 0, 0, kt + 2);
    DLION_GEMM_PHASE_MATH(0)
    read_a(1, 1);
    if (more) {
      stage(0, 1, 0, kt + 2);
      vm_wait8();
    } else {
      vm_wait0();
    }
    DLION_GEMM_PHASE_MATH(1)
    read_a(1, 2);
    if (more) stage(1, 0, 1, kt + 3);
    DLION_GEMM_PHASE_MATH(2)
    read_a(1, 3);
    if (more) {
      stage(1, 1, 1, kt + 3);
      vm_wait6();
    }
    DLION_GEMM_PHASE_MATH(3)
  }
#undef DLION_GEMM_PHASE_MATH
#undef DLION_GEMM_MFMA
  if (wr == 0) __builtin_amdgcn_s_barrier();
  DLION_STAMP(st_[2])

  uint8_t* reg = lds + w * (128 * 128);
  float bv[4][4] = {};
  if constexpr (EPI == 1) {
#pragma unroll
    for (int nt = 0; nt < 4; ++nt)
#pragma unroll
      for (int j = 0; j < 4; ++j) {
        const int n = n0 + wc * 64 + nt * 16 + 4 * (lane >> 4) + j;
        bv[nt][j] = n < g.N ? bf16_to_f32(g.bias[n]) : 0.f;
      }
  }
  const int row_base = m0 + wr * 128;
  const int col_base = n0 + wc * 64;

  auto park = [&](auto fn) {
#pragma unroll
    for (int mt = 0; mt < 8; ++mt)
#pragma unroll
      for (int nt = 0; nt < 4; ++nt) {
        const int row = mt * 16 + (lane & 15);
        const int col = nt * 16 + 4 * (lane >> 4);
        const int chunk = (col >> 3) ^ (row & 7);
        const uint32_t lo = static_cast<uint32_t>(fn(acc[mt][nt][0], nt, 0)) |
                            (static_cast<uint32_t>(fn(acc[mt][nt][1], nt, 1)) << 16);
        const uint32_t hi = static_cast<uint32_t>(fn(acc[mt][nt][2], nt, 2)) |
                            (static_cast<uint32_t>(fn(acc[mt][nt][3], nt, 3)) << 16);
        *reinterpret_cast<uint2*>(reg + row * 128 + chunk * 16 + (col & 7) * 2) = make_uint2(lo, hi);
      }
    asm volatile("s_waitcnt lgkmcnt(0)" ::: "memory");
    __builtin_amdgcn_wave_barrier();
  };
  const int ch = lane & 7;
  const int gn = col_base + ch * 8;

  if constexpr (EPI <= 1) {
    park([&](float v, int nt, int j) { return __builtin_bit_cast(uint16_t, static_cast<__bf16>(v + bv[nt][j])); });
    DLION_STAMP(st_[3])
#pragma unroll
    for (int i = 0; i < 16; ++i) {
      const int row = i * 8 + (lane >> 3);
      const uint4 v = *reinterpret_cast<const uint4*>(reg + row * 128 + ((ch ^ (row & 7)) << 4));
      const int gm = row_base + row;
      if (gm < g.M && gn < g.N) st16<false>(g.C + (int64_t)gm * g.ldc + gn, v);
    }
    if constexpr (STAMP) {
      DLION_STAMP(st_[4])
      DLION_RSTAMP(st_[6])
      if (tid < 8) g.stamps[static_cast<int64_t>(blockIdx.x) * 8 + tid] = tid < 7 ? st_[tid < 7 ? tid : 0] : 0ull;
    }
  } else if constexpr (EPI <= 3 || EPI == 6 || EPI == 7) {
    park([&](float v, int, int) { return __builtin_bit_cast(uint16_t, static_cast<__bf16>(v)); });
    float b8[8];
    if (gn < g.N) {
      Elem<kBF16>::load8(g.bias + gn, b8);
    } else {
#pragma unroll
      for (int j = 0; j < 8; ++j) b8[j] = 0.f;
    }
#pragma unroll 4
    for (int i = 0; i < 16; ++i) {
      const int row = i * 8 + (lane >> 3);
      const uint4 v = *reinterpret_cast<const uint4*>(reg + row * 128 + ((ch ^ (row & 7)) << 4));
      const int gm = row_base + row;
      if (gm < g.M && gn < g.N) {
        float z[8];
        Elem<kBF16>::load8(reinterpret_cast<const uint16_t*>(&v), z);
        bf16x8 hb;
        if constexpr (EPI <= 3) {
          st16<kNtAux>(g.aux + (int64_t)gm * g.ldaux + gn, v);
#pragma unroll
          for (int j = 0; j < 8; ++j) hb[j] = static_cast<__bf16>(gelu_f(z[j] + b8[j], EPI == 3));
        } else {
          bf16x8 db;
#pragma unroll
          for (int j = 0; j < 8; ++j) {
            float gv, dgv;
            gelu_and_grad(z[j] + b8[j], EPI == 7, gv, dgv);
            hb[j] = static_cast<__bf16>(gv);
            db[j] = static_cast<__bf16>(dgv);
          }
          st16<kNtAux>(g.aux + (int64_t)gm * g.ldaux + gn, db);
        }
        st16<kNtC>(g.C + (int64_t)gm * g.ldc + gn, hb);
      }
    }
  } else {
    uint4 zr[16];
#pragma unroll
    for (int i = 0; i < 16; ++i) {
      const int gm = min(row_base + i * 8 + (lane >> 3), g.M - 1);
      zr[i] = gn < g.N ? ld16<kNtAux>(g.aux + (int64_t)gm * g.ldaux + gn) : make_uint4(0, 0, 0, 0);
    }
    park([&](float v, int, int) { return __builtin_bit_cast(uint16_t, static_cast<__bf16>(v)); });
    float b8[8], cs[8];
#pragma unroll
    for (int j = 0; j < 8; ++j) cs[j] = 0.f;
    if (EPI != 8 && gn < g.N) {
      Elem<kBF16>::load8(g.bias + gn, b8);
    } else {
#pragma unroll
      for (int j = 0; j < 8; ++j) b8[j] = 0.f;
    }
#pragma unroll
    for (int i = 0; i < 16; ++i) {
      const int row = i * 8 + (lane >> 3);
      const uint4 v = *reinterpret_cast<const uint4*>(reg + row * 128 + ((ch ^ (row & 7)) << 4));
      const int gm = row_base + row;
      if (gm < g.M && gn < g.N) {
        float gv[8], z[8], o[8];
        Elem<kBF16>::load8(reinterpret_cast<const uint16_t*>(&v), gv);
        Elem<kBF16>::load8(reinterpret_cast<const uint16_t*>(&zr[i]), z);
        bf16x8 ob;
#pragma unroll
        for (int j = 0; j < 8; ++j) {
          if constexpr (EPI == 8) {
            o[j] = gv[j] * z[j];
          } else {
            o[j] = gv[j] * gelu_grad(z[j] + b8[j], EPI == 5);
          }
          ob[j] = static_cast<__bf16>(o[j]);
          cs[j] += static_cast<float>(ob[j]);
        }
        st16<kNtC>(g.C + (int64_t)gm * g.ldc + gn, ob);
      }
    }
#pragma unroll
    for (int j = 0; j < 8; ++j) {
      cs[j] += __shfl_xor(cs[j], 8);
      cs[j] += __shfl_xor(cs[j], 16);
      cs[j] += __shfl_xor(cs[j], 32);
    }
    if (lane < 8 && gn < g.N) {
      float* dst = g.part + (int64_t)(2 * tm + wr) * g.N + gn;
      *reinterpret_cast<float4*>(dst) = make_float4(cs[0], cs[1], cs[2], cs[3]);
      *reinterpret_cast<float4*>(dst + 4) = make_float4(cs[4], cs[5], cs[6], cs[7]);
    }
  }
}

}

hipError_t launch_gemm_nt_stamped(const void* A, int lda, const void* B, int ldb, void* C, int ldc, int M, int N, int K,
                                  unsigned long long* stamps, hipStream_t st) {
  if (K % 128 != 0 || N % 8 != 0) return hipErrorInvalidValue;
  GemmArgs g{};
  g.A = static_cast<const uint16_t*>(A);
  g.B = static_cast<const uint16_t*>(B);
  g.C = static_cast<uint16_t*>(C);
  g.lda = lda;
  g.ldb = ldb;
  g.ldc = ldc;
  g.M = M;
  g.N = N;
  g.K = K;
  g.tiles_m = (M + kBM - 1) / kBM;
  g.tiles_n = (N + kBN - 1) / kBN;
  g.stamps = stamps;
  hipLaunchKernelGGL((gemm_nt_kernel<0, true>), dim3(g.tiles_m * g.tiles_n), dim3(512), 0, st, g);
  return hipGetLastError();
}


hipError_t launch_gemm_nt(const void* A, int lda, const void* B, int ldb, void* C, int ldc, const void* bias,
                          void* aux, int ldaux, int M, int N, int K, int epi, float* part, hipStream_t st) {
  if (M <= 0 || N <= 0) return hipSuccess;
  if (K % 128 != 0 || N % 8 != 0 || lda % 8 != 0 || ldb % 8 != 0 || ldc % 8 != 0) return hipErrorInvalidValue;
  if ((int64_t)M * lda >= (1ll << 31) || (int64_t)N * ldb >= (1ll << 31)) return hipErrorInvalidValue;
  if (epi >= 2 && (aux == nullptr || ldaux % 8 != 0)) return hipErrorInvalidValue;
  if (epi >= 1 && epi != 8 && (bias == nullptr || reinterpret_cast<uintptr_t>(bias) % 16 != 0))
    return hipErrorInvalidValue;
  if ((epi == 4 || epi == 5 || epi == 8) && (part == nullptr || reinterpret_cast<uintptr_t>(part) % 16 != 0))
    return hipErrorInvalidValue;
  GemmArgs g;
  g.A = static_cast<const uint16_t*>(A);
  g.B = static_cast<const uint16_t*>(B);
  g.C = static_cast<uint16_t*>(C);
  g.bias = static_cast<const uint16_t*>(bias);
  g.aux = static_cast<uint16_t*>(aux);
  g.part = part;
  g.lda = lda;
  g.ldb = ldb;
  g.ldc = ldc;
  g.ldaux = ldaux;
  g.M = M;
  g.N = N;
  g.K = K;
  g.tiles_m = (M + kBM - 1) / kBM;
  g.tiles_n = (N + kBN - 1) / kBN;
  const dim3 grid(g.tiles_m * g.tiles_n), block(512);
  switch (epi) {
    case 0: hipLaunchKernelGGL(gemm_nt_kernel<0>, grid, block, 0, st, g); break;
    case 1: hipLaunchKernelGGL(gemm_nt_kernel<1>, grid, block, 0, st, g); break;
    case 2: hipLaunchKernelGGL(gemm_nt_kernel<2>, grid, block, 0, st, g); break;
    case 3: hipLaunchKernelGGL(gemm_nt_kernel<3>, grid, block, 0, st, g); break;
    case 4: hipLaunchKernelGGL(gemm_nt_kernel<4>, grid, block, 0, st, g); break;
    case 5: hipLaunchKernelGGL(gemm_nt_kernel<5>, grid, block, 0, st, g); break;
    case 6: hipLaunchKernelGGL(gemm_nt_kernel<6>, grid, block, 0, st, g); break;
    case 7: hipLaunchKernelGGL(gemm_nt_kernel<7>, grid, block, 0, st, g); break;
    case 8: hipLaunchKernelGGL(gemm_nt_kernel<8>, grid, block, 0, st, g); break;
    default: return hipErrorInvalidValue;
  }
  return hipGetLastError();
}

}
```

### distributed_lion_pytorch_amd/csrc/kernels.h

```cpp
#pragma once
#include <hip/hip_runtime.h>
#include <stdint.h>

#include "attention.h"

namespace dlion {

hipError_t launch_lion_local(int dt, const int64_t* seg, const int64_t* chunks, int64_t n_chunks, float decay,
                             float neg_lr, float b1, float omb1, float b2, float omb2, const float* gscale,
                             hipStream_t st, int rounding = 0, uint32_t rkey = 0, int64_t cbase = 0);
hipError_t launch_lion_encode(int dt, const int64_t* seg, const int64_t* chunks, int64_t n_chunks, uint8_t* bits,
                              float b1, float omb1, float b2, float omb2, int update_m, int stochastic, float rr,
                              uint64_t seed, uint32_t step, const float* gscale, hipStream_t st,
                              int64_t cbase = 0);
hipError_t launch_grad_sumsq(int dt, const int64_t* seg, const int64_t* chunks, int64_t n_chunks, float* partial,
                             hipStream_t st);
hipError_t launch_clip_coef(const float* partial, int64_t n, float max_norm, float* out, hipStream_t st);
hipError_t launch_lion_vote_apply(int dt, const int64_t* seg, const int64_t* chunks, int64_t n_chunks,
                                  const uint8_t* planes, int64_t plane_stride, const uint8_t* alive, int world,
                                  int mode, int tie, const uint8_t* neg, float decay, float neg_lr, const uint8_t* own,
                                  unsigned long long* agree, hipStream_t st, int rounding = 0, uint32_t rkey = 0,
                                  int64_t cbase = 0);
hipError_t launch_vote_reduce(const uint8_t* recv, int64_t nbytes, const uint8_t* alive, int world, int tie,
                              uint8_t* out, uint8_t* neg_out, unsigned long long* ties, hipStream_t st);
hipError_t launch_vote_count(const uint8_t* recv, int64_t nbytes, const uint8_t* alive, int world, uint8_t* out,
                             unsigned long long* ties, hipStream_t st);

hipError_t launch_attn_fwd(const AttnArgs& a, int D, bool drop, hipStream_t st);
hipError_t launch_attn_bwd(const AttnArgs& a, int D, bool drop, hipStream_t st);

hipError_t launch_add_norm_fwd(const void* x, const void* y, const void* bias, const void* gamma, const void* beta,
                               void* xo, void* h, float* mean, float* rstd, int64_t rows, int C, float eps, bool rms,
                               uint32_t seed, uint32_t thresh16, float inv_keep, hipStream_t st);
hipError_t launch_add_norm_bwd(const void* dh, const void* dxo_in, const void* xo, const void* gamma, const float* mean,
                               const float* rstd, void* dx, void* dy, float* part, int parts, int64_t rows, int C,
                               bool rms, uint32_t seed, uint32_t thresh16, float inv_keep, hipStream_t st);

hipError_t launch_bias_gelu_fwd(const void* z, const void* b, void* h, int64_t rows, int N, bool exact,
                                hipStream_t st);
hipError_t launch_bias_gelu_bwd(const void* dh, const void* z, const void* b, void* dz, float* dbpart, int parts,
                                int64_t rows, int N, bool exact, hipStream_t st);
hipError_t launch_swiglu_fwd(const void* g, const void* u, void* h, int64_t rows, int64_t F, int64_t ld_in,
                             hipStream_t st);
hipError_t launch_swiglu_fwd_t(const void* g, const void* u, void* h, void* ht, int64_t rows, int64_t F,
                               int64_t ld_in, hipStream_t st);
hipError_t launch_swiglu_bwd_t(const void* dh, const void* g, const void* u, void* dgu, void* dgut, int64_t rows,
                               int64_t F, int64_t ld_in, hipStream_t st);
hipError_t launch_swiglu_bwd(const void* dh, const void* g, const void* u, void* dg, void* du, int64_t rows,
                             int64_t F, int64_t ld_in, int64_t ld_out, hipStream_t st);
hipError_t launch_rope(const void* x, const void* cos, const void* sin, void* y, int64_t rows, int T, int H, int D,
                       bool inverse, int64_t x_ld, int64_t y_ld, hipStream_t st);
hipError_t launch_qk_norm_rope_fwd(const void* x, const void* gamma_a, const void* gamma_b, const void* cos,
                                   const void* sin, void* y, float* rstd, int64_t rows, int T, int Hx, int D,
                                   int split, float eps, int64_t x_ld, hipStream_t st);
hipError_t launch_qk_norm_rope_bwd(void* g, const void* x, const float* rstd, const void* gamma_a, const void* gamma_b,
                                   const void* cos, const void* sin, float* part, int parts, int64_t rows, int T,
                                   int Hx, int D, int split, int64_t g_ld, int64_t x_ld, hipStream_t st);
hipError_t launch_sum_partials(const float* part, int S, int64_t n, int64_t ld, void* out, bool accumulate,
                               hipStream_t st, const float* scale = nullptr);
hipError_t launch_colsum(const void* x, float* part, int parts, int64_t rows, int N, hipStream_t st);
hipError_t launch_sum_partials_multi(const float* const* ptrs, const int64_t* rows, const int64_t* lds, int nseg,
                                     int64_t n, void* out, bool accumulate, hipStream_t st);
int sum_partials_split_factor(int64_t n, int64_t total_rows);
hipError_t launch_transpose_pad(const void* x, int64_t R, int64_t C, int64_t ldx, void* out, int64_t Rp,
                                hipStream_t st);
hipError_t launch_sum_partials_split(const float* const* ptrs, const int64_t* rows, const int64_t* lds, int nseg,
                                     int64_t n, int Y, float* scratch, void* out, bool accumulate, const float* scale,
                                     hipStream_t st);

hipError_t launch_gemm_nt(const void* A, int lda, const void* B, int ldb, void* C, int ldc, const void* bias,
                          void* aux, int ldaux, int M, int N, int K, int epi, float* part, hipStream_t st);

hipError_t launch_embed_fwd(const int64_t* ids, const void* wte, const void* wpe, void* out, int64_t n, int C, int T,
                            int64_t V, uint32_t seed, uint32_t thresh16, float inv_keep, int32_t* err, hipStream_t st);
constexpr int kIndexErrEmbed = 1, kIndexErrLabel = 2;
hipError_t launch_index_check(const int64_t* ids, int64_t n, int64_t hi, int64_t ignore, int32_t* err, int code,
                              hipStream_t st);
hipError_t launch_embed_bwd(const void* dx, const int64_t* sid, const int64_t* perm, void* dwte, void* dwpe, int64_t n,
                            int C, int T, int64_t V, int pos_accumulate, uint32_t seed, uint32_t thresh16,
                            float inv_keep, hipStream_t st);
hipError_t launch_scale_acc(const void* x, const float* s, void* y, int64_t n, int accumulate, hipStream_t st);

hipError_t launch_gemm_tn(const void* const* P, const void* const* Q, int nseg, int64_t seg_rows, int ldp, int ldq,
                          float* C, int M, int N, int splits, bool accumulate, hipStream_t st, void* Cb = nullptr);

hipError_t launch_gemm_nt_stamped(const void* A, int lda, const void* B, int ldb, void* C, int ldc, int M, int N, int K,
                                  unsigned long long* stamps, hipStream_t st);

hipError_t launch_lora_rows(const void* in, int64_t ldin, const void* w, void* out, int64_t rows, int K, int r,
                            float scale, uint32_t seed, uint32_t thresh16, float inv_keep, hipStream_t st);
hipError_t launch_lora_up(const void* o, int64_t ldo, const void* u, const void* b, void* out, int64_t rows, int N, int r,
                          float s, hipStream_t st);
int lora_cols_parts(int64_t rows, int N);
hipError_t launch_lora_cols(const void* g, int64_t ldg, const void* y, const void* a, void* dx, float* part, int64_t rows,
                            int N, int r, int parts, int mode, float yscale, uint32_t seed, uint32_t thresh16,
                            float inv_keep, hipStream_t st);
bool lora_wide_rank(int r);
hipError_t launch_lora_rows_wide(const void* in, int64_t ldin, const void* w, void* out, int64_t rows, int K, int r,
                                 float scale, uint32_t seed, uint32_t thresh16, float inv_keep, hipStream_t st);
hipError_t launch_lora_up_wide(const void* o, int64_t ldo, const void* u, const void* b, void* out, int64_t rows, int N,
                               int r, float s, hipStream_t st);
int lora_cols_parts_wide(int64_t rows, int N, int r);
hipError_t launch_lora_cols_wide(const void* g, int64_t ldg, const void* y, const void* a, void* dx, float* part,
                                 int64_t rows, int N, int r, int parts, int mode, float yscale, uint32_t seed,
                                 uint32_t thresh16, float inv_keep, hipStream_t st);

hipError_t launch_quant4(int dt, const void* w, const float* code, uint8_t* q, float* absmax, int64_t n,
                         hipStream_t st);
hipError_t launch_dequant4(int dt, const uint8_t* q, const float* absmax, const float* code, void* out, int64_t n,
                           hipStream_t st);
hipError_t launch_dequant4_t(int dt, const uint8_t* q, const float* absmax, const float* code, void* out, int N, int K,
                             int64_t ldo, hipStream_t st);

hipError_t launch_softmax_xent(int dt, void* logits, const int64_t* labels, int64_t n, int64_t vp, int v, float* loss,
                               int variant, hipStream_t st);
hipError_t launch_softmax_xent_opts(int dt, void* logits, const int64_t* labels, int64_t n, int64_t vp, int v,
                                    float* loss, float eps, float zeta, int variant, hipStream_t st);

hipError_t launch_lm_score(int dt, const void* logits, const int64_t* labels, int64_t n, int64_t vp, int v, float eps,
                           float zeta, float* row_loss, float* row_lse, int* pred, int* rank, hipStream_t st);

}
```

Measured before the change: 1.072 million tokens/s.

## Add selectable GEMM tile geometries with a cost-model picker for wave quantization

```diff
diff --git a/distributed_lion_pytorch_amd/csrc/bindings.cpp b/distributed_lion_pytorch_amd/csrc/bindings.cpp
--- a/distributed_lion_pytorch_amd/csrc/bindings.cpp
+++ b/distributed_lion_pytorch_amd/csrc/bindings.cpp
@@ -5,6 +5,8 @@
 
 #include <hip/hip_runtime.h>
 
+#include <array>
+#include <atomic>
 #include <cstdlib>
 #include <string>
 #include <tuple>
@@ -818,8 +820,28 @@
          a.size(0) * a.stride(0) < (1ll << 31) && b.size(0) * b.stride(0) < (1ll << 31);
 }
 
+int gemm_num_cus(int dev) {
+  static std::array<std::atomic<int>, 64> cus{};
+  const bool cached = dev >= 0 && dev < static_cast<int>(cus.size());
+  int n = cached ? cus[dev].load(std::memory_order_relaxed) : 0;
+  if (n == 0) {
+    check_hip(hipDeviceGetAttribute(&n, hipDeviceAttributeMultiprocessorCount, dev), "gemm_num_cus");
+    if (cached) cus[dev].store(n, std::memory_order_relaxed);
+  }
+  return n;
+}
+
+dlion::NtTile gemm_nt_tile_for(const Tensor& a, const Tensor& b, int64_t epi) {
+  return dlion::gemm_nt_tile(static_cast<int>(a.size(0)), static_cast<int>(b.size(0)), static_cast<int>(a.size(1)),
+                             static_cast<int>(epi), gemm_num_cus(a.get_device()));
+}
+
+Tensor gemm_nt_part(const Tensor& a, const Tensor& b, dlion::NtTile tile) {
+  return at::empty({2 * ((a.size(0) + tile.bm - 1) / tile.bm), b.size(0)}, a.options().dtype(at::kFloat));
+}
+
 void gemm_nt_launch(const Tensor& a, const Tensor& b, const Tensor& c, const Tensor* bias, const Tensor* aux,
-                    int64_t epi, const Tensor* part = nullptr) {
+                    int64_t epi, const Tensor* part = nullptr, const dlion::NtTile* forced = nullptr) {
   check_gemm_operand(a, "a");
   check_gemm_operand(b, "b");
   check_gemm_operand(c, "out");
@@ -835,10 +857,11 @@
     check_gemm_operand(*aux, "aux");
     TORCH_CHECK(aux->size(0) == c.size(0) && aux->size(1) == c.size(1), "dlion gemm: aux must match the output shape");
   }
+  const dlion::NtTile tile = forced ? *forced : gemm_nt_tile_for(a, b, epi);
   if (part) {
     TORCH_CHECK(part->is_cuda() && part->scalar_type() == at::kFloat && part->is_contiguous() &&
-                    part->size(0) == 2 * ((a.size(0) + 255) / 256) && part->size(1) == b.size(0),
-                "dlion gemm: part must be fp32 [2 * ceil(M / 256), N]");
+                    part->size(0) == 2 * ((a.size(0) + tile.bm - 1) / tile.bm) && part->size(1) == b.size(0),
+                "dlion gemm: part must be fp32 [2 * ceil(M / tile rows), N]");
   }
   const c10::DeviceGuard g(a.device());
   check_hip(dlion::launch_gemm_nt(a.data_ptr(), static_cast<int>(a.stride(0)), b.data_ptr(),
@@ -846,8 +869,33 @@
                                   bias ? bias->data_ptr() : nullptr, aux ? aux->data_ptr() : nullptr,
                                   aux ? static_cast<int>(aux->stride(0)) : 0, static_cast<int>(a.size(0)),
                                   static_cast<int>(b.size(0)), static_cast<int>(a.size(1)), static_cast<int>(epi),
-                                  part ? part->data_ptr<float>() : nullptr, cur_stream()),
+                                  part ? part->data_ptr<float>() : nullptr, tile, cur_stream()),
             "gemm_nt");
+}
+
+std::tuple<int64_t, int64_t> gemm_nt_tile(int64_t M, int64_t N, int64_t K, int64_t epi) {
+  int dev = 0;
+  check_hip(hipGetDevice(&dev), "gemm_nt_tile");
+  const int cus = gemm_num_cus(dev);
+  const dlion::NtTile t = dlion::gemm_nt_tile(static_cast<int>(M), static_cast<int>(N), static_cast<int>(K),
+                                              static_cast<int>(epi), cus);
+  return {t.bm, t.bn};
+}
+
+std::tuple<int64_t, int64_t> gemm_nt_tile_pick(int64_t M, int64_t N, int64_t K, int64_t epi, int64_t num_cus) {
+  const dlion::NtTile t = dlion::pick_nt_tile(static_cast<int>(M), static_cast<int>(N), static_cast<int>(K),
+                                              static_cast<int>(epi), static_cast<int>(num_cus));
+  return {t.bm, t.bn};
+}
+
+double gemm_nt_tile_cost(int64_t M, int64_t N, int64_t K, int64_t epi, int64_t num_cus, int64_t bm, int64_t bn) {
+  return dlion::nt_tile_cost_us(static_cast<int>(M), static_cast<int>(N), static_cast<int>(K), static_cast<int>(epi),
+                                static_cast<int>(num_cus), dlion::NtTile{static_cast<int>(bm), static_cast<int>(bn)});
+}
+
+void set_gemm_nt_tile(int64_t bm, int64_t bn) {
+  TORCH_CHECK(dlion::set_gemm_nt_tile(static_cast<int>(bm), static_cast<int>(bn)),
+              "dlion gemm: tile must be (0, 0), (256, 256), (320, 256), (320, 192) or (256, 192)");
 }
 
 Tensor gemm_nt(const Tensor& a, const Tensor& b, const std::optional<Tensor>& bias) {
@@ -1020,22 +1068,30 @@
             "scale_acc");
 }
 
-Tensor gemm_nt_stamped(const Tensor& a, const Tensor& b, const Tensor& stamps) {
+Tensor gemm_nt_stamped(const Tensor& a, const Tensor& b, const Tensor& stamps, const std::optional<Tensor>& bias) {
   check_gemm_operand(a, "a");
   check_gemm_operand(b, "b");
   TORCH_CHECK(gemm_nt_supported(a, b), "dlion gemm: unsupported shape");
-  const int64_t blocks = ((a.size(0) + 255) / 256) * ((b.size(0) + 255) / 256);
+  const int epi = bias.has_value() ? 6 : 0;
+  const dlion::NtTile tile = gemm_nt_tile_for(a, b, epi);
+  const int64_t blocks = ((a.size(0) + tile.bm - 1) / tile.bm) * ((b.size(0) + tile.bn - 1) / tile.bn);
   TORCH_CHECK(stamps.is_cuda() && stamps.scalar_type() == at::kLong && stamps.is_contiguous() &&
                   stamps.numel() >= blocks * 8,
               "dlion gemm: stamps must be int64 [blocks, 8]");
+  if (bias.has_value()) {
+    TORCH_CHECK(bias->is_cuda() && bias->scalar_type() == at::kBFloat16 && bias->is_contiguous() &&
+                    bias->numel() == b.size(0),
+                "dlion gemm: bias must be a contiguous bf16 [N] tensor");
+  }
   auto c = at::empty({a.size(0), b.size(0)}, a.options());
+  Tensor aux = bias.has_value() ? at::empty_like(c) : Tensor();
   const c10::DeviceGuard g(a.device());
-  check_hip(dlion::launch_gemm_nt_stamped(a.data_ptr(), static_cast<int>(a.stride(0)), b.data_ptr(),
-                                          static_cast<int>(b.stride(0)), c.data_ptr(), static_cast<int>(c.stride(0)),
-                                          static_cast<int>(a.size(0)), static_cast<int>(b.size(0)),
-                                          static_cast<int>(a.size(1)),
-                                          reinterpret_cast<unsigned long long*>(stamps.data_ptr<int64_t>()),
-                                          cur_stream()),
+  check_hip(dlion::launch_gemm_nt_stamped(
+                a.data_ptr(), static_cast<int>(a.stride(0)), b.data_ptr(), static_cast<int>(b.stride(0)), c.data_ptr(),
+                static_cast<int>(c.stride(0)), bias.has_value() ? bias->data_ptr() : nullptr,
+                bias.has_value() ? aux.data_ptr() : nullptr, bias.has_value() ? static_cast<int>(aux.stride(0)) : 0,
+                static_cast<int>(a.size(0)), static_cast<int>(b.size(0)), static_cast<int>(a.size(1)), epi, tile,
+                reinterpret_cast<unsigned long long*>(stamps.data_ptr<int64_t>()), cur_stream()),
             "gemm_nt_stamped");
   return c;
 }
@@ -1049,16 +1105,18 @@
 
 std::tuple<Tensor, Tensor> gemm_nt_dmul(const Tensor& a, const Tensor& b, const Tensor& d) {
   auto dz = at::empty({a.size(0), b.size(0)}, a.options());
-  auto part = at::empty({2 * ((a.size(0) + 255) / 256), b.size(0)}, a.options().dtype(at::kFloat));
-  gemm_nt_launch(a, b, dz, nullptr, &d, 8, &part);
+  const dlion::NtTile tile = gemm_nt_tile_for(a, b, 8);
+  auto part = gemm_nt_part(a, b, tile);
+  gemm_nt_launch(a, b, dz, nullptr, &d, 8, &part, &tile);
   return {dz, part};
 }
 
 std::tuple<Tensor, Tensor> gemm_nt_dgelu(const Tensor& a, const Tensor& b, const Tensor& bias, const Tensor& z,
                                          bool exact) {
   auto dz = at::empty({a.size(0), b.size(0)}, a.options());
-  auto part = at::empty({2 * ((a.size(0) + 255) / 256), b.size(0)}, a.options().dtype(at::kFloat));
-  gemm_nt_launch(a, b, dz, &bias, &z, exact ? 5 : 4, &part);
+  const dlion::NtTile tile = gemm_nt_tile_for(a, b, exact ? 5 : 4);
+  auto part = gemm_nt_part(a, b, tile);
+  gemm_nt_launch(a, b, dz, &bias, &z, exact ? 5 : 4, &part, &tile);
   return {dz, part};
 }
 
@@ -1270,7 +1328,11 @@
   m.def("gemm_nt_dgelu(Tensor a, Tensor b, Tensor bias, Tensor z, bool exact) -> (Tensor, Tensor)");
   m.def("gemm_nt_gelu_d(Tensor a, Tensor b, Tensor bias, bool exact) -> (Tensor, Tensor)");
   m.def("gemm_nt_dmul(Tensor a, Tensor b, Tensor d) -> (Tensor, Tensor)");
-  m.def("gemm_nt_stamped(Tensor a, Tensor b, Tensor(a!) stamps) -> Tensor");
+  m.def("gemm_nt_stamped(Tensor a, Tensor b, Tensor(a!) stamps, Tensor? bias=None) -> Tensor");
+  m.def("gemm_nt_tile(int M, int N, int K, int epi) -> (int, int)", &gemm_nt_tile);
+  m.def("gemm_nt_tile_pick(int M, int N, int K, int epi, int num_cus) -> (int, int)", &gemm_nt_tile_pick);
+  m.def("gemm_nt_tile_cost(int M, int N, int K, int epi, int num_cus, int bm, int bn) -> float", &gemm_nt_tile_cost);
+  m.def("set_gemm_nt_tile(int bm, int bn) -> ()", &set_gemm_nt_tile);
   m.def("embed_fwd(Tensor ids, Tensor wte, Tensor wpe, float p, int seed, Tensor(a!)? err=None) -> Tensor");
   m.def("index_check_(Tensor ids, int hi, int ignore, Tensor(a!) err, int code) -> ()");
   m.def(
diff --git a/distributed_lion_pytorch_amd/csrc/gemm.hip b/distributed_lion_pytorch_amd/csrc/gemm.hip
--- a/distributed_lion_pytorch_amd/csrc/gemm.hip
+++ b/distributed_lion_pytorch_amd/csrc/gemm.hip
@@ -1,6 +1,8 @@
 #include "common.h"
+#include "kernels.h"
 
 #include <algorithm>
+#include <type_traits>
 
 namespace dlion {
 
@@ -9,9 +11,18 @@
 typedef __bf16 bf16x8 __attribute__((ext_vector_type(8)));
 typedef float f32x4 __attribute__((ext_vector_type(4)));
 
-constexpr int kBM = 256, kBN = 256, kBK = 64;
+constexpr int kBK = 64;
 constexpr int kHalf = 128 * kBK * 2;
-constexpr int kLds = 8 * kHalf;
+constexpr int kPiece = 64 * kBK * 2;
+
+template <int RB, int NS>
+struct Geo {
+  static constexpr int BM = 64 * RB, BN = 64 * NS, WM = 32 * RB, WN = 16 * NS;
+  static constexpr bool kLegacy = RB == 4 && NS == 4;
+  static constexpr int kLds = 2 * (RB + NS) * kPiece > 8 * kHalf ? 2 * (RB + NS) * kPiece : 8 * kHalf;
+};
+template <int V>
+using ic = std::integral_constant<int, V>;
 
 struct GemmArgs {
   const uint16_t* A;
@@ -32,6 +43,11 @@
 __device__ __forceinline__ void vm_wait8() { asm volatile("s_waitcnt vmcnt(8)" ::: "memory"); }
 __device__ __forceinline__ void vm_wait2() { asm volatile("s_waitcnt vmcnt(2)" ::: "memory"); }
 __device__ __forceinline__ void vm_wait0() { asm volatile("s_waitcnt vmcnt(0)" ::: "memory"); }
+template <int N>
+__device__ __forceinline__ void vm_wait() {
+  static_assert(N >= 0 && N < 64, "vmcnt is a 6-bit field");
+  asm volatile("s_waitcnt vmcnt(%0)" ::"n"(N) : "memory");
+}
 
 __device__ __forceinline__ void glds16(const uint16_t* base, uint32_t boff, uint8_t* dst) {
   const uint8_t* src = reinterpret_cast<const uint8_t*>(base) + boff;
@@ -76,12 +92,15 @@
     __builtin_amdgcn_sched_barrier(0);                                              \
   }
 
-template <int EPI, bool STAMP = false>
+template <int EPI, bool STAMP = false, int RB = 4, int NS = 4>
 __global__ void __launch_bounds__(512, 1) gemm_nt_kernel(const GemmArgs g) {
+  using G = Geo<RB, NS>;
+  constexpr int kBM = G::BM, kBN = G::BN;
+  constexpr bool kLegacy = G::kLegacy;
   unsigned long long st_[7] = {0, 0, 0, 0, 0, 0, 0};
   DLION_RSTAMP(st_[5])
   DLION_STAMP(st_[0])
-  __shared__ __attribute__((aligned(16))) uint8_t lds[kLds];
+  __shared__ __attribute__((aligned(16))) uint8_t lds[G::kLds];
 
   const int tid = threadIdx.x;
   const int w = __builtin_amdgcn_readfirstlane(tid >> 6), lane = tid & 63;
@@ -102,7 +121,22 @@
   const int m0 = tm * kBM, n0 = tn * kBN;
 
   Stage st;
-  {
+  uint32_t poff[RB + NS];
+  if constexpr (!kLegacy) {
+    const int pc = lane & 7;
+    const int lr = 8 * w + (lane >> 3);
+    const int c = pc ^ ((lr >> 1) & 7);
+#pragma unroll
+    for (int p = 0; p < RB; ++p) {
+      const int ra = min(m0 + (lr >> 5) * G::WM + 32 * p + (lr & 31), g.M - 1);
+      poff[p] = static_cast<uint32_t>(ra * g.lda + c * 8) * 2u;
+    }
+#pragma unroll
+    for (int j = 0; j < NS; ++j) {
+      const int rb = min(n0 + 64 * j + lr, g.N - 1);
+      poff[RB + j] = static_cast<uint32_t>(rb * g.ldb + c * 8) * 2u;
+    }
+  } else {
     const int pc = lane & 7;
 #pragma unroll
     for (int pi = 0; pi < 2; ++pi) {
@@ -129,33 +163,41 @@
     glds16(base, st.off[ab][half][0], dst);
     glds16(base, st.off[ab][half][1], dst + 1024);
   };
+  auto pstage = [&](int idx, int dbuf, int kt) {
+    const uint16_t* base = (idx < RB ? Ag : Bg) + kt * kBK;
+    asm volatile("" : "+s"(base));
+    uint8_t* dst = lds + (dbuf * (RB + NS) + idx) * kPiece + w * 1024;
+    asm volatile("" : "+v"(poff[idx]));
+    glds16(base, poff[idx], dst);
+  };
 
   const int lr16 = lane & 15;
   const int swz = (lr16 >> 1) & 7;
   const int foff0 = lr16 * 128 + (((lane >> 4) ^ swz) << 4);
   const int foff1 = lr16 * 128 + (((4 + (lane >> 4)) ^ swz) << 4);
-  const int a_row_base = wr * 64 * 128;
-  const int b_base_off = ((wc >> 1) * kHalf) + (wc & 1) * 64 * 128;
-
-  f32x4 acc[8][4];
-#pragma unroll
-  for (int i = 0; i < 8; ++i)
-#pragma unroll
-    for (int j = 0; j < 4; ++j) acc[i][j] = f32x4{0.f, 0.f, 0.f, 0.f};
-
-  bf16x8 bfr[4][2];
+  const int a_row_base = kLegacy ? wr * 64 * 128 : wr * 32 * 128;
+  const int b_base_off = kLegacy ? ((wc >> 1) * kHalf) + (wc & 1) * 64 * 128 : RB * kPiece + wc * G::WN * 128;
+
+  f32x4 acc[2 * RB][NS];
+#pragma unroll
+  for (int i = 0; i < 2 * RB; ++i)
+#pragma unroll
+    for (int j = 0; j < NS; ++j) acc[i][j] = f32x4{0.f, 0.f, 0.f, 0.f};
+
+  bf16x8 bfr[NS][2];
   bf16x8 afr[2][2];
 
   auto read_b = [&](int dbuf) {
-    const uint8_t* base = lds + slot(dbuf, 1, 0) + b_base_off;
-#pragma unroll
-    for (int nt = 0; nt < 4; ++nt) {
+    const uint8_t* base = lds + (kLegacy ? slot(dbuf, 1, 0) : dbuf * (RB + NS) * kPiece) + b_base_off;
+#pragma unroll
+    for (int nt = 0; nt < NS; ++nt) {
       bfr[nt][0] = *reinterpret_cast<const bf16x8*>(base + nt * 16 * 128 + foff0);
       bfr[nt][1] = *reinterpret_cast<const bf16x8*>(base + nt * 16 * 128 + foff1);
     }
   };
   auto read_a = [&](int dbuf, int p) {
-    const uint8_t* base = lds + slot(dbuf, 0, p >> 1) + a_row_base + (2 * (p & 1)) * 16 * 128;
+    const uint8_t* base = lds + (kLegacy ? slot(dbuf, 0, p >> 1) : (dbuf * (RB + NS) + p) * kPiece) + a_row_base +
+                          (kLegacy ? (2 * (p & 1)) * 16 * 128 : 0);
 #pragma unroll
     for (int mt = 0; mt < 2; ++mt) {
       afr[mt][0] = *reinterpret_cast<const bf16x8*>(base + mt * 16 * 128 + foff0);
@@ -167,7 +209,7 @@
   do {                                                                           \
     __builtin_amdgcn_s_setprio(1);                                               \
     _Pragma("unroll") for (int mt = 0; mt < 2; ++mt)                             \
-    _Pragma("unroll") for (int nt = 0; nt < 4; ++nt)                             \
+    _Pragma("unroll") for (int nt = 0; nt < NS; ++nt)                            \
     _Pragma("unroll") for (int s = 0; s < 2; ++s)                                \
       acc[2 * (P) + mt][nt] = mfma16(bfr[nt][s], afr[mt][s], acc[2 * (P) + mt][nt]); \
     __builtin_amdgcn_s_setprio(0);                                               \
@@ -184,60 +226,114 @@
   const int nk = g.K / kBK;
   const int nit = nk / 2;
 
-  stage(1, 0, 0, 0);
-  stage(1, 1, 0, 0);
-  stage(0, 0, 0, 0);
-  stage(0, 1, 0, 0);
-  stage(1, 0, 1, 1);
-  stage(1, 1, 1, 1);
-  vm_wait6();
-  __builtin_amdgcn_s_barrier();
-  if (wr == 1) __builtin_amdgcn_s_barrier();
-  DLION_STAMP(st_[1])
-
-  for (int it = 0; it < nit; ++it) {
-    const int kt = 2 * it;
-    const bool more = it + 1 < nit;
-    read_b(0);
-    read_a(0, 0);
-    stage(0, 0, 1, kt + 1);
-    DLION_GEMM_PHASE_MATH(0)
-    read_a(0, 1);
-    stage(0, 1, 1, kt + 1);
-    vm_wait8();
-    DLION_GEMM_PHASE_MATH(1)
-    read_a(0, 2);
-    if (more) stage(1, 0, 0, kt + 2);
-    DLION_GEMM_PHASE_MATH(2)
-    read_a(0, 3);
-    if (more) {
-      stage(1, 1, 0, kt + 2);
-      vm_wait6();
-    } else {
-      vm_wait2();
-    }
-    DLION_GEMM_PHASE_MATH(3)
-    read_b(1);
-    read_a(1, 0);
-    if (more) stage(0, 0, 0, kt + 2);
-    DLION_GEMM_PHASE_MATH(0)
-    read_a(1, 1);
-    if (more) {
-      stage(0, 1, 0, kt + 2);
+  if constexpr (kLegacy) {
+    stage(1, 0, 0, 0);
+    stage(1, 1, 0, 0);
+    stage(0, 0, 0, 0);
+    stage(0, 1, 0, 0);
+    stage(1, 0, 1, 1);
+    stage(1, 1, 1, 1);
+    vm_wait6();
+    __builtin_amdgcn_s_barrier();
+    if (wr == 1) __builtin_amdgcn_s_barrier();
+    DLION_STAMP(st_[1])
+
+    for (int it = 0; it < nit; ++it) {
+      const int kt = 2 * it;
+      const bool more = it + 1 < nit;
+      read_b(0);
+      read_a(0, 0);
+      stage(0, 0, 1, kt + 1);
+      DLION_GEMM_PHASE_MATH(0)
+      read_a(0, 1);
+      stage(0, 1, 1, kt + 1);
       vm_wait8();
-    } else {
-      vm_wait0();
-    }
-    DLION_GEMM_PHASE_MATH(1)
-    read_a(1, 2);
-    if (more) stage(1, 0, 1, kt + 3);
-    DLION_GEMM_PHASE_MATH(2)
-    read_a(1, 3);
-    if (more) {
-      stage(1, 1, 1, kt + 3);
-      vm_wait6();
-    }
-    DLION_GEMM_PHASE_MATH(3)
+      DLION_GEMM_PHASE_MATH(1)
+      read_a(0, 2);
+      if (more) stage(1, 0, 0, kt + 2);
+      DLION_GEMM_PHASE_MATH(2)
+      read_a(0, 3);
+      if (more) {
+        stage(1, 1, 0, kt + 2);
+        vm_wait6();
+      } else {
+        vm_wait2();
+      }
+      DLION_GEMM_PHASE_MATH(3)
+      read_b(1);
+      read_a(1, 0);
+      if (more) stage(0, 0, 0, kt + 2);
+      DLION_GEMM_PHASE_MATH(0)
+      read_a(1, 1);
+      if (more) {
+        stage(0, 1, 0, kt + 2);
+        vm_wait8();
+      } else {
+        vm_wait0();
+      }
+      DLION_GEMM_PHASE_MATH(1)
+      read_a(1, 2);
+      if (more) stage(1, 0, 1, kt + 3);
+      DLION_GEMM_PHASE_MATH(2)
+      read_a(1, 3);
+      if (more) {
+        stage(1, 1, 1, kt + 3);
+        vm_wait6();
+      }
+      DLION_GEMM_PHASE_MATH(3)
+    }
+  } else {
+    constexpr int L = RB + NS;
+    static_assert(RB >= 4 && L <= 2 * RB, "B restages start in phase >= 2 and end in phase RB-1");
+#pragma unroll
+    for (int j = 0; j < NS; ++j) pstage(RB + j, 0, 0);
+#pragma unroll
+    for (int q = 0; q < RB; ++q) pstage(q, 0, 0);
+#pragma unroll
+    for (int j = 0; j < NS; ++j) pstage(RB + j, 1, 1);
+    vm_wait<RB - 1 + NS>();
+    __builtin_amdgcn_s_barrier();
+    if (wr == 1) __builtin_amdgcn_s_barrier();
+    DLION_STAMP(st_[1])
+
+    auto phase = [&](auto P_, auto D_, auto A1_, auto B2_, int kt) {
+      constexpr int P = decltype(P_)::value, D = decltype(D_)::value;
+      constexpr bool A1 = decltype(A1_)::value != 0, B2 = decltype(B2_)::value != 0;
+      if constexpr (P == 0) read_b(D);
+      read_a(D, P);
+      auto load = [&](auto I_) {
+        constexpr int i = decltype(I_)::value;
+        if constexpr (i < RB) {
+          if constexpr (A1) pstage(i, D ^ 1, kt + 1);
+        } else if constexpr (i < L) {
+          if constexpr (B2) pstage(i, D, kt + 2);
+        }
+      };
+      load(ic<2 * P>{});
+      load(ic<2 * P + 1>{});
+      constexpr int na = 2 * (P + 1) < RB ? 2 * (P + 1) : RB;
+      constexpr int nb = 2 * (P + 1) - RB < 0 ? 0 : (2 * (P + 1) - RB > NS ? NS : 2 * (P + 1) - RB);
+      constexpr int here = (A1 ? na : 0) + (B2 ? nb : 0);
+      if constexpr (P < RB - 1) {
+        vm_wait<(RB - 2 - P) + (A1 ? NS : 0) + here>();
+      } else if constexpr (A1) {
+        vm_wait<here - 1>();
+      }
+      DLION_GEMM_PHASE_MATH(P)
+    };
+    auto ktile = [&](auto D_, auto A1_, auto B2_, int kt) {
+      phase(ic<0>{}, D_, A1_, B2_, kt);
+      phase(ic<1>{}, D_, A1_, B2_, kt);
+      phase(ic<2>{}, D_, A1_, B2_, kt);
+      phase(ic<3>{}, D_, A1_, B2_, kt);
+      if constexpr (RB == 5) phase(ic<4>{}, D_, A1_, B2_, kt);
+    };
+    for (int it = 0; it + 1 < nit; ++it) {
+      ktile(ic<0>{}, ic<1>{}, ic<1>{}, 2 * it);
+      ktile(ic<1>{}, ic<1>{}, ic<1>{}, 2 * it + 1);
+    }
+    ktile(ic<0>{}, ic<1>{}, ic<0>{}, nk - 2);
+    ktile(ic<1>{}, ic<0>{}, ic<0>{}, nk - 1);
   }
 #undef DLION_GEMM_PHASE_MATH
 #undef DLION_GEMM_MFMA
@@ -245,31 +341,32 @@
   DLION_STAMP(st_[2])
 
   uint8_t* reg = lds + w * (128 * 128);
-  float bv[4][4] = {};
+  float bv[NS][4] = {};
   if constexpr (EPI == 1) {
 #pragma unroll
-    for (int nt = 0; nt < 4; ++nt)
+    for (int nt = 0; nt < NS; ++nt)
 #pragma unroll
       for (int j = 0; j < 4; ++j) {
-        const int n = n0 + wc * 64 + nt * 16 + 4 * (lane >> 4) + j;
+        const int n = n0 + wc * G::WN + nt * 16 + 4 * (lane >> 4) + j;
         bv[nt][j] = n < g.N ? bf16_to_f32(g.bias[n]) : 0.f;
       }
   }
-  const int row_base = m0 + wr * 128;
-  const int col_base = n0 + wc * 64;
-
-  auto park = [&](auto fn) {
-#pragma unroll
-    for (int mt = 0; mt < 8; ++mt)
-#pragma unroll
-      for (int nt = 0; nt < 4; ++nt) {
+  const int row_base = m0 + wr * G::WM;
+  const int col_base = n0 + wc * G::WN;
+
+  auto park = [&](auto MT0_, auto NMT_, auto fn) {
+    constexpr int MT0 = decltype(MT0_)::value, NMT = decltype(NMT_)::value;
+#pragma unroll
+    for (int mt = 0; mt < NMT; ++mt)
+#pragma unroll
+      for (int nt = 0; nt < NS; ++nt) {
         const int row = mt * 16 + (lane & 15);
         const int col = nt * 16 + 4 * (lane >> 4);
         const int chunk = (col >> 3) ^ (row & 7);
-        const uint32_t lo = static_cast<uint32_t>(fn(acc[mt][nt][0], nt, 0)) |
-                            (static_cast<uint32_t>(fn(acc[mt][nt][1], nt, 1)) << 16);
-        const uint32_t hi = static_cast<uint32_t>(fn(acc[mt][nt][2], nt, 2)) |
-                            (static_cast<uint32_t>(fn(acc[mt][nt][3], nt, 3)) << 16);
+        const uint32_t lo = static_cast<uint32_t>(fn(acc[MT0 + mt][nt][0], nt, 0)) |
+                            (static_cast<uint32_t>(fn(acc[MT0 + mt][nt][1], nt, 1)) << 16);
+        const uint32_t hi = static_cast<uint32_t>(fn(acc[MT0 + mt][nt][2], nt, 2)) |
+                            (static_cast<uint32_t>(fn(acc[MT0 + mt][nt][3], nt, 3)) << 16);
         *reinterpret_cast<uint2*>(reg + row * 128 + chunk * 16 + (col & 7) * 2) = make_uint2(lo, hi);
       }
     asm volatile("s_waitcnt lgkmcnt(0)" ::: "memory");
@@ -277,137 +374,249 @@
   };
   const int ch = lane & 7;
   const int gn = col_base + ch * 8;
-
-  if constexpr (EPI <= 1) {
-    park([&](float v, int nt, int j) { return __builtin_bit_cast(uint16_t, static_cast<__bf16>(v + bv[nt][j])); });
-    DLION_STAMP(st_[3])
-#pragma unroll
-    for (int i = 0; i < 16; ++i) {
-      const int row = i * 8 + (lane >> 3);
-      const uint4 v = *reinterpret_cast<const uint4*>(reg + row * 128 + ((ch ^ (row & 7)) << 4));
-      const int gm = row_base + row;
-      if (gm < g.M && gn < g.N) st16<false>(g.C + (int64_t)gm * g.ldc + gn, v);
-    }
-    if constexpr (STAMP) {
-      DLION_STAMP(st_[4])
-      DLION_RSTAMP(st_[6])
-      if (tid < 8) g.stamps[static_cast<int64_t>(blockIdx.x) * 8 + tid] = tid < 7 ? st_[tid < 7 ? tid : 0] : 0ull;
-    }
-  } else if constexpr (EPI <= 3 || EPI == 6 || EPI == 7) {
-    park([&](float v, int, int) { return __builtin_bit_cast(uint16_t, static_cast<__bf16>(v)); });
-    float b8[8];
-    if (gn < g.N) {
-      Elem<kBF16>::load8(g.bias + gn, b8);
+  const int eN = g.N;
+  auto col_ok_ = [&]() { return (NS == 4 || ch < 2 * NS) && gn < eN; };
+#define col_ok col_ok_()
+  float b8[8], cs[8];
+
+  const int eM = g.M, eldc = g.ldc, eldaux = g.ldaux;
+  uint16_t* const cC = g.C + gn;
+  uint16_t* const caux = g.aux + gn;
+  const uint16_t* const cbias = g.bias + gn;
+  auto pass = [&](auto MT0_, auto NMT_) {
+    constexpr int MT0 = decltype(MT0_)::value, NMT = decltype(NMT_)::value;
+    const int prow = row_base + MT0 * 16;
+    if constexpr (MT0 > 0) __builtin_amdgcn_wave_barrier();
+    if constexpr (EPI <= 1) {
+      park(MT0_, NMT_,
+           [&](float v, int nt, int j) { return __builtin_bit_cast(uint16_t, static_cast<__bf16>(v + bv[nt][j])); });
+      if constexpr (MT0 == 0) { DLION_STAMP(st_[3]) }
+#pragma unroll
+      for (int i = 0; i < 2 * NMT; ++i) {
+        const int row = i * 8 + (lane >> 3);
+        const uint4 v = *reinterpret_cast<const uint4*>(reg + row * 128 + ((ch ^ (row & 7)) << 4));
+        const int gm = prow + row;
+        if (gm < eM && col_ok) st16<false>(cC + (int64_t)gm * eldc, v);
+      }
+    } else if constexpr (EPI <= 3 || EPI == 6 || EPI == 7) {
+      park(MT0_, NMT_, [&](float v, int, int) { return __builtin_bit_cast(uint16_t, static_cast<__bf16>(v)); });
+      if constexpr (MT0 == 0) {
+        DLION_STAMP(st_[3])
+        if (col_ok) {
+          Elem<kBF16>::load8(cbias, b8);
+        } else {
+#pragma unroll
+          for (int j = 0; j < 8; ++j) b8[j] = 0.f;
+        }
+      }
+#pragma unroll 4
+      for (int i = 0; i < 2 * NMT; ++i) {
+        const int row = i * 8 + (lane >> 3);
+        const uint4 v = *reinterpret_cast<const uint4*>(reg + row * 128 + ((ch ^ (row & 7)) << 4));
+        const int gm = prow + row;
+        if (gm < eM && col_ok) {
+          float z[8];
+          Elem<kBF16>::load8(reinterpret_cast<const uint16_t*>(&v), z);
+          bf16x8 hb;
+          if constexpr (EPI <= 3) {
+            st16<kNtAux>(caux + (int64_t)gm * eldaux, v);
+#pragma unroll
+            for (int j = 0; j < 8; ++j) hb[j] = static_cast<__bf16>(gelu_f(z[j] + b8[j], EPI == 3));
+          } else {
+            bf16x8 db;
+#pragma unroll
+            for (int j = 0; j < 8; ++j) {
+              float gv, dgv;
+              gelu_and_grad(z[j] + b8[j], EPI == 7, gv, dgv);
+              hb[j] = static_cast<__bf16>(gv);
+              db[j] = static_cast<__bf16>(dgv);
+            }
+            st16<kNtAux>(caux + (int64_t)gm * eldaux, db);
+          }
+          st16<kNtC>(cC + (int64_t)gm * eldc, hb);
+        }
+      }
     } else {
-#pragma unroll
-      for (int j = 0; j < 8; ++j) b8[j] = 0.f;
-    }
-#pragma unroll 4
-    for (int i = 0; i < 16; ++i) {
-      const int row = i * 8 + (lane >> 3);
-      const uint4 v = *reinterpret_cast<const uint4*>(reg + row * 128 + ((ch ^ (row & 7)) << 4));
-      const int gm = row_base + row;
-      if (gm < g.M && gn < g.N) {
-        float z[8];
-        Elem<kBF16>::load8(reinterpret_cast<const uint16_t*>(&v), z);
-        bf16x8 hb;
-        if constexpr (EPI <= 3) {
-          st16<kNtAux>(g.aux + (int64_t)gm * g.ldaux + gn, v);
-#pragma unroll
-          for (int j = 0; j < 8; ++j) hb[j] = static_cast<__bf16>(gelu_f(z[j] + b8[j], EPI == 3));
+      uint4 zr[2 * NMT];
+#pragma unroll
+      for (int i = 0; i < 2 * NMT; ++i) {
+        const int gm = min(prow + i * 8 + (lane >> 3), eM - 1);
+        zr[i] = col_ok ? ld16<kNtAux>(caux + (int64_t)gm * eldaux) : make_uint4(0, 0, 0, 0);
+      }
+      park(MT0_, NMT_, [&](float v, int, int) { return __builtin_bit_cast(uint16_t, static_cast<__bf16>(v)); });
+      if constexpr (MT0 == 0) {
+        DLION_STAMP(st_[3])
+#pragma unroll
+        for (int j = 0; j < 8; ++j) cs[j] = 0.f;
+        if (EPI != 8 && col_ok) {
+          Elem<kBF16>::load8(cbias, b8);
         } else {
-          bf16x8 db;
+#pragma unroll
+          for (int j = 0; j < 8; ++j) b8[j] = 0.f;
+        }
+      }
+#pragma unroll
+      for (int i = 0; i < 2 * NMT; ++i) {
+        const int row = i * 8 + (lane >> 3);
+        const uint4 v = *reinterpret_cast<const uint4*>(reg + row * 128 + ((ch ^ (row & 7)) << 4));
+        const int gm = prow + row;
+        if (gm < eM && col_ok) {
+          float gv[8], z[8], o[8];
+          Elem<kBF16>::load8(reinterpret_cast<const uint16_t*>(&v), gv);
+          Elem<kBF16>::load8(reinterpret_cast<const uint16_t*>(&zr[i]), z);
+          bf16x8 ob;
 #pragma unroll
           for (int j = 0; j < 8; ++j) {
-            float gv, dgv;
-            gelu_and_grad(z[j] + b8[j], EPI == 7, gv, dgv);
-            hb[j] = static_cast<__bf16>(gv);
-            db[j] = static_cast<__bf16>(dgv);
+            if constexpr (EPI == 8) {
+              o[j] = gv[j] * z[j];
+            } else {
+              o[j] = gv[j] * gelu_grad(z[j] + b8[j], EPI == 5);
+            }
+            ob[j] = static_cast<__bf16>(o[j]);
+            cs[j] += static_cast<float>(ob[j]);
           }
-          st16<kNtAux>(g.aux + (int64_t)gm * g.ldaux + gn, db);
+          st16<kNtC>(cC + (int64_t)gm * eldc, ob);
         }
-        st16<kNtC>(g.C + (int64_t)gm * g.ldc + gn, hb);
-      }
-    }
+      }
+    }
+  };
+  if constexpr (RB == 4) {
+    pass(ic<0>{}, ic<8>{});
   } else {
-    uint4 zr[16];
-#pragma unroll
-    for (int i = 0; i < 16; ++i) {
-      const int gm = min(row_base + i * 8 + (lane >> 3), g.M - 1);
-      zr[i] = gn < g.N ? ld16<kNtAux>(g.aux + (int64_t)gm * g.ldaux + gn) : make_uint4(0, 0, 0, 0);
-    }
-    park([&](float v, int, int) { return __builtin_bit_cast(uint16_t, static_cast<__bf16>(v)); });
-    float b8[8], cs[8];
-#pragma unroll
-    for (int j = 0; j < 8; ++j) cs[j] = 0.f;
-    if (EPI != 8 && gn < g.N) {
-      Elem<kBF16>::load8(g.bias + gn, b8);
-    } else {
-#pragma unroll
-      for (int j = 0; j < 8; ++j) b8[j] = 0.f;
-    }
-#pragma unroll
-    for (int i = 0; i < 16; ++i) {
-      const int row = i * 8 + (lane >> 3);
-      const uint4 v = *reinterpret_cast<const uint4*>(reg + row * 128 + ((ch ^ (row & 7)) << 4));
-      const int gm = row_base + row;
-      if (gm < g.M && gn < g.N) {
-        float gv[8], z[8], o[8];
-        Elem<kBF16>::load8(reinterpret_cast<const uint16_t*>(&v), gv);
-        Elem<kBF16>::load8(reinterpret_cast<const uint16_t*>(&zr[i]), z);
-        bf16x8 ob;
-#pragma unroll
-        for (int j = 0; j < 8; ++j) {
-          if constexpr (EPI == 8) {
-            o[j] = gv[j] * z[j];
-          } else {
-            o[j] = gv[j] * gelu_grad(z[j] + b8[j], EPI == 5);
-          }
-          ob[j] = static_cast<__bf16>(o[j]);
-          cs[j] += static_cast<float>(ob[j]);
-        }
-        st16<kNtC>(g.C + (int64_t)gm * g.ldc + gn, ob);
-      }
-    }
+    pass(ic<0>{}, ic<5>{});
+    pass(ic<5>{}, ic<5>{});
+  }
+  if constexpr (EPI == 4 || EPI == 5 || EPI == 8) {
 #pragma unroll
     for (int j = 0; j < 8; ++j) {
       cs[j] += __shfl_xor(cs[j], 8);
       cs[j] += __shfl_xor(cs[j], 16);
       cs[j] += __shfl_xor(cs[j], 32);
     }
-    if (lane < 8 && gn < g.N) {
+    if (lane < 8 && col_ok) {
       float* dst = g.part + (int64_t)(2 * tm + wr) * g.N + gn;
       *reinterpret_cast<float4*>(dst) = make_float4(cs[0], cs[1], cs[2], cs[3]);
       *reinterpret_cast<float4*>(dst + 4) = make_float4(cs[4], cs[5], cs[6], cs[7]);
     }
   }
-}
-
-}
-
-hipError_t launch_gemm_nt_stamped(const void* A, int lda, const void* B, int ldb, void* C, int ldc, int M, int N, int K,
+#undef col_ok
+  if constexpr (STAMP) {
+    DLION_STAMP(st_[4])
+    DLION_RSTAMP(st_[6])
+    if (tid < 8) g.stamps[static_cast<int64_t>(blockIdx.x) * 8 + tid] = tid < 7 ? st_[tid < 7 ? tid : 0] : 0ull;
+  }
+}
+
+}
+
+namespace {
+
+constexpr double kPrologueUs = 1.9;
+constexpr double kHandoverPlainUs = 2.6, kHandoverGeluUs = 6.5;
+constexpr double kKtileUs256x256 = 1.362, kKtileUs320x256 = 1.333, kKtileUs320x192 = 1.426, kKtileUs256x192 = 1.45;
+constexpr double kEpiPlainUs = 2.66, kEpiPlain192Us = 3.3, kEpiGeluUs = 7.3;
+constexpr double kMinGain = 0.03;
+
+constexpr NtTile kTiles[4] = {{256, 256}, {320, 256}, {320, 192}, {256, 192}};
+NtTile g_tile_override = {0, 0};
+
+double ktile_us(NtTile t) {
+  if (t.bm == 256) return t.bn == 256 ? kKtileUs256x256 : kKtileUs256x192;
+  return t.bn == 256 ? kKtileUs320x256 : kKtileUs320x192;
+}
+
+}
+
+double nt_tile_cost_us(int M, int N, int K, int epi, int num_cus, NtTile t) {
+  const int64_t tiles = static_cast<int64_t>((M + t.bm - 1) / t.bm) * ((N + t.bn - 1) / t.bn);
+  const int64_t rounds = (tiles + num_cus - 1) / std::max(num_cus, 1);
+  const double area = static_cast<double>(t.bm) * t.bn / (256.0 * 256.0);
+  const double epi_us = epi <= 1 ? (t.bn == 256 ? kEpiPlainUs : kEpiPlain192Us) : kEpiGeluUs;
+  const double hand_us = epi <= 1 ? kHandoverPlainUs : kHandoverGeluUs;
+  return static_cast<double>(rounds) * (kPrologueUs + area * (K / 64 * ktile_us(t) + epi_us) + hand_us);
+}
+
+NtTile pick_nt_tile(int M, int N, int K, int epi, int num_cus) {
+  NtTile best = kTiles[0];
+  const int64_t tiles = static_cast<int64_t>((M + 255) / 256) * ((N + 255) / 256);
+  if (num_cus <= 0 || 2 * tiles < num_cus) return best;
+  const double base = nt_tile_cost_us(M, N, K, epi, num_cus, best);
+  double best_cost = base * (1.0 - kMinGain);
+  auto slots = [&](NtTile t) {
+    const int64_t n = static_cast<int64_t>((M + t.bm - 1) / t.bm) * ((N + t.bn - 1) / t.bn);
+    return (n + num_cus - 1) / num_cus * t.bm * t.bn;
+  };
+  for (int i = 1; i < 3; ++i) {
+    if (M % kTiles[i].bm != 0 || N % kTiles[i].bn != 0) continue;
+    if (slots(kTiles[i]) > slots(kTiles[0])) continue;
+    const double c = nt_tile_cost_us(M, N, K, epi, num_cus, kTiles[i]);
+    if (c < best_cost) {
+      best_cost = c;
+      best = kTiles[i];
+    }
+  }
+  return best;
+}
+
+NtTile gemm_nt_tile(int M, int N, int K, int epi, int num_cus) {
+  return g_tile_override.bm ? g_tile_override : pick_nt_tile(M, N, K, epi, num_cus);
+}
+
+bool set_gemm_nt_tile(int bm, int bn) {
+  if (bm == 0 && bn == 0) {
+    g_tile_override = {0, 0};
+    return true;
+  }
+  for (const NtTile& t : kTiles)
+    if (t.bm == bm && t.bn == bn) {
+      g_tile_override = t;
+      return true;
+    }
+  return false;
+}
+
+namespace {
+
+template <int EPI, bool STAMP>
+hipError_t launch_geo(GemmArgs& g, NtTile t, hipStream_t st) {
+  g.tiles_m = (g.M + t.bm - 1) / t.bm;
+  g.tiles_n = (g.N + t.bn - 1) / t.bn;
+  const dim3 grid(g.tiles_m * g.tiles_n), block(512);
+  if (t.bm == 256 && t.bn == 256) hipLaunchKernelGGL((gemm_nt_kernel<EPI, STAMP, 4, 4>), grid, block, 0, st, g);
+  else if (t.bm == 320 && t.bn == 256) hipLaunchKernelGGL((gemm_nt_kernel<EPI, STAMP, 5, 4>), grid, block, 0, st, g);
+  else if (t.bm == 320 && t.bn == 192) hipLaunchKernelGGL((gemm_nt_kernel<EPI, STAMP, 5, 3>), grid, block, 0, st, g);
+  else if (t.bm == 256 && t.bn == 192) hipLaunchKernelGGL((gemm_nt_kernel<EPI, STAMP, 4, 3>), grid, block, 0, st, g);
+  else return hipErrorInvalidValue;
+  return hipGetLastError();
+}
+
+}
+
+hipError_t launch_gemm_nt_stamped(const void* A, int lda, const void* B, int ldb, void* C, int ldc, const void* bias,
+                                  void* aux, int ldaux, int M, int N, int K, int epi, NtTile tile,
                                   unsigned long long* stamps, hipStream_t st) {
   if (K % 128 != 0 || N % 8 != 0) return hipErrorInvalidValue;
+  if (epi != 0 && (epi != 6 || bias == nullptr || aux == nullptr)) return hipErrorInvalidValue;
   GemmArgs g{};
   g.A = static_cast<const uint16_t*>(A);
   g.B = static_cast<const uint16_t*>(B);
   g.C = static_cast<uint16_t*>(C);
+  g.bias = static_cast<const uint16_t*>(bias);
+  g.aux = static_cast<uint16_t*>(aux);
   g.lda = lda;
   g.ldb = ldb;
   g.ldc = ldc;
+  g.ldaux = ldaux;
   g.M = M;
   g.N = N;
   g.K = K;
-  g.tiles_m = (M + kBM - 1) / kBM;
-  g.tiles_n = (N + kBN - 1) / kBN;
   g.stamps = stamps;
-  hipLaunchKernelGGL((gemm_nt_kernel<0, true>), dim3(g.tiles_m * g.tiles_n), dim3(512), 0, st, g);
-  return hipGetLastError();
-}
-
+  return epi == 0 ? launch_geo<0, true>(g, tile, st) : launch_geo<6, true>(g, tile, st);
+}
 
 hipError_t launch_gemm_nt(const void* A, int lda, const void* B, int ldb, void* C, int ldc, const void* bias,
-                          void* aux, int ldaux, int M, int N, int K, int epi, float* part, hipStream_t st) {
+                          void* aux, int ldaux, int M, int N, int K, int epi, float* part, NtTile tile,
+                          hipStream_t st) {
   if (M <= 0 || N <= 0) return hipSuccess;
   if (K % 128 != 0 || N % 8 != 0 || lda % 8 != 0 || ldb % 8 != 0 || ldc % 8 != 0) return hipErrorInvalidValue;
   if ((int64_t)M * lda >= (1ll << 31) || (int64_t)N * ldb >= (1ll << 31)) return hipErrorInvalidValue;
@@ -416,7 +625,7 @@
     return hipErrorInvalidValue;
   if ((epi == 4 || epi == 5 || epi == 8) && (part == nullptr || reinterpret_cast<uintptr_t>(part) % 16 != 0))
     return hipErrorInvalidValue;
-  GemmArgs g;
+  GemmArgs g{};
   g.A = static_cast<const uint16_t*>(A);
   g.B = static_cast<const uint16_t*>(B);
   g.C = static_cast<uint16_t*>(C);
@@ -430,22 +639,18 @@
   g.M = M;
   g.N = N;
   g.K = K;
-  g.tiles_m = (M + kBM - 1) / kBM;
-  g.tiles_n = (N + kBN - 1) / kBN;
-  const dim3 grid(g.tiles_m * g.tiles_n), block(512);
   switch (epi) {
-    case 0: hipLaunchKernelGGL(gemm_nt_kernel<0>, grid, block, 0, st, g); break;
-    case 1: hipLaunchKernelGGL(gemm_nt_kernel<1>, grid, block, 0, st, g); break;
-    case 2: hipLaunchKernelGGL(gemm_nt_kernel<2>, grid, block, 0, st, g); break;
-    case 3: hipLaunchKernelGGL(gemm_nt_kernel<3>, grid, block, 0, st, g); break;
-    case 4: hipLaunchKernelGGL(gemm_nt_kernel<4>, grid, block, 0, st, g); break;
-    case 5: hipLaunchKernelGGL(gemm_nt_kernel<5>, grid, block, 0, st, g); break;
-    case 6: hipLaunchKernelGGL(gemm_nt_kernel<6>, grid, block, 0, st, g); break;
-    case 7: hipLaunchKernelGGL(gemm_nt_kernel<7>, grid, block, 0, st, g); break;
-    case 8: hipLaunchKernelGGL(gemm_nt_kernel<8>, grid, block, 0, st, g); break;
+    case 0: return launch_geo<0, false>(g, tile, st);
+    case 1: return launch_geo<1, false>(g, tile, st);
+    case 2: return launch_geo<2, false>(g, tile, st);
+    case 3: return launch_geo<3, false>(g, tile, st);
+    case 4: return launch_geo<4, false>(g, tile, st);
+    case 5: return launch_geo<5, false>(g, tile, st);
+    case 6: return launch_geo<6, false>(g, tile, st);
+    case 7: return launch_geo<7, false>(g, tile, st);
+    case 8: return launch_geo<8, false>(g, tile, st);
     default: return hipErrorInvalidValue;
   }
-  return hipGetLastError();
-}
-
-}
+}
+
+}
diff --git a/distributed_lion_pytorch_amd/csrc/kernels.h b/distributed_lion_pytorch_amd/csrc/kernels.h
--- a/distributed_lion_pytorch_amd/csrc/kernels.h
+++ b/distributed_lion_pytorch_amd/csrc/kernels.h
@@ -68,8 +68,16 @@
                                      int64_t n, int Y, float* scratch, void* out, bool accumulate, const float* scale,
                                      hipStream_t st);
 
+struct NtTile {
+  int bm, bn;
+};
+NtTile gemm_nt_tile(int M, int N, int K, int epi, int num_cus);
+NtTile pick_nt_tile(int M, int N, int K, int epi, int num_cus);
+double nt_tile_cost_us(int M, int N, int K, int epi, int num_cus, NtTile t);
+bool set_gemm_nt_tile(int bm, int bn);
 hipError_t launch_gemm_nt(const void* A, int lda, const void* B, int ldb, void* C, int ldc, const void* bias,
-                          void* aux, int ldaux, int M, int N, int K, int epi, float* part, hipStream_t st);
+                          void* aux, int ldaux, int M, int N, int K, int epi, float* part, NtTile tile,
+                          hipStream_t st);
 
 hipError_t launch_embed_fwd(const int64_t* ids, const void* wte, const void* wpe, void* out, int64_t n, int C, int T,
                             int64_t V, uint32_t seed, uint32_t thresh16, float inv_keep, int32_t* err, hipStream_t st);
@@ -84,7 +92,8 @@
 hipError_t launch_gemm_tn(const void* const* P, const void* const* Q, int nseg, int64_t seg_rows, int ldp, int ldq,
                           float* C, int M, int N, int splits, bool accumulate, hipStream_t st, void* Cb = nullptr);
 
-hipError_t launch_gemm_nt_stamped(const void* A, int lda, const void* B, int ldb, void* C, int ldc, int M, int N, int K,
+hipError_t launch_gemm_nt_stamped(const void* A, int lda, const void* B, int ldb, void* C, int ldc, const void* bias,
+                                  void* aux, int ldaux, int M, int N, int K, int epi, NtTile tile,
                                   unsigned long long* stamps, hipStream_t st);
 
 hipError_t launch_lora_rows(const void* in, int64_t ldin, const void* w, void* out, int64_t rows, int K, int r,
```

Measured after the change: 1.048 million tokens/s. -2.2%, worse.
